# ghar1821/Chronoclust

Hardware: AMD Instinct MI355X
Metric: points clustered/sec (20-dim) (higher is better)
Workload: dtype f64; 1 GPU; C2: 1 timepoint, 1000000x20 synthetic blobs (seed 42+rank), 5000 microclusters; exact sequential semantics; online + offline phases per step; one independent st; points=1000000, dim=20, microclusters=5000, clusters=5000, streams=1

## Files before the change

### chronoclust_amd/_lib.py

```python
import ctypes as C
import os

import numpy as np

from . import build as _build

PCORE, OUTLIER = 0, 1
MAX_DIM = 1024

_ERRORS = {-1: "no HIP device / HIP runtime error", -2: "bad argument", -3: "non-finite input", -4: "out of memory",
           -5: "internal error", -6: "exchange between ranks failed"}


class ChronoclustHipError(RuntimeError):
    pass


class CcParams(C.Structure):
    _fields_ = [("eps_sq", C.c_double), ("delta_sq", C.c_double), ("k", C.c_double), ("beta", C.c_double),
                ("mu", C.c_double), ("omicron", C.c_double), ("ups_eps", C.c_double), ("ups_eps_sq", C.c_double),
                ("delta", C.c_double), ("pi", C.c_int32), ("pad", C.c_int32)]


class CcTuning(C.Structure):
# ... 165 lines not shown
        self._cofactors = None
        if transform is not None:
            if not isinstance(transform, ListTransform):
                raise ValueError("ListMode: transform must be a ListTransform")
            self._cofactors = transform.cofactors(self.shape[1])

    def __len__(self):
        return self.n

    def descriptor(self):
        return CcListMode(self._bytes.ctypes.data if self._bytes.size else None, self.n, self.src_cols,
                          LIST_DTYPES[self.dtype.newbyteorder("=")], LM_SWAPPED if self.swapped else 0, self.shape[1],
                          self.columns.ctypes.data_as(C.POINTER(C.c_int32)),
                          None if self.masks is None else self.masks.ctypes.data_as(C.POINTER(C.c_uint32)))

    def transform_descriptor(self):
        t = self.transform
        if t is None:
            return None
        return CcListTransform(t.m, 0, t.comp_cols.ctypes.data_as(C.POINTER(C.c_int32)) if t.m else None,
                               t.comp.ctypes.data_as(C.POINTER(C.c_double)) if t.m else None,
                               None if self._cofactors is None else self._cofactors.ctypes.data_as(C.POINTER(C.c_double)))

    def __array__(self, dtype=None, copy=None):
        rec = np.frombuffer(self._bytes, dtype=self.dtype, count=self.n * self.src_cols).reshape(self.n, self.src_cols)
        native = self.dtype.newbyteorder("=")
        out = rec[:, self.columns]
        if self.masks is not None:
            out = out.astype(native) & self.masks.astype(native)
        if self.transform is not None:
            out = self._host_transform(rec, out.astype(np.float64))
        else:
            out = out.astype(np.float32 if self.dtype.itemsize == 4 and self.dtype.kind == "f" else np.float64)
        return out if dtype is None else out.astype(dtype, copy=False)

    def _host_transform(self, rec, out):
        t = self.transform
        native = self.dtype.newbyteorder("=")
        cols = self.columns.tolist()
        xs = []
        for c in t.comp_cols.tolist():
            x = rec[:, c].astype(native)
            if self.masks is not None and c in cols:
                x = x & self.masks[cols.index(c)].astype(native)
            xs.append(x.astype(np.float64))
        for k, c in enumerate(cols):
            hit = np.flatnonzero(t.comp_cols == c)
            if hit.size:
                i = int(hit[0])
                v = xs[0] * t.comp[0, i]
                for j in range(1, t.m):
                    v = v + xs[j] * t.comp[j, i]
                out[:, k] = v
        if self._cofactors is not None:
            with np.errstate(all="ignore"):
                for k, cf in enumerate(self._cofactors.tolist()):
                    if cf > 0:
                        out[:, k] = np.arcsinh(out[:, k] / cf)
        return out


class CcRelaxedStats(C.Structure):
    _fields_ = [("super_steps", C.c_int64), ("minibatch_points", C.c_int64), ("deferred_points", C.c_int64),
                ("reserved", C.c_int64 * 5)]


_dp = C.POINTER(C.c_double)
_fp = C.POINTER(C.c_float)
_i64p = C.POINTER(C.c_int64)
_i32p = C.POINTER(C.c_int32)
_i8p = C.POINTER(C.c_int8)
_vp = C.POINTER(CcPointsView)
_lp = C.POINTER(CcListMode)
_xp = C.POINTER(CcListTransform)

SYMBOLS = {
    "cc_create": (C.c_int, [C.c_int, C.POINTER(C.c_void_p)]),
    "cc_destroy": (None, [C.c_void_p]),
    "cc_last_error": (C.c_char_p, [C.c_void_p]),
    "cc_set_tuning": (C.c_int, [C.c_void_p, C.POINTER(CcTuning)]),
    "cc_reset": (C.c_int, [C.c_void_p]),
    "cc_set_params": (C.c_int, [C.c_void_p, C.POINTER(CcParams)]),
    "cc_decay_downgrade": (C.c_int, [C.c_void_p, C.c_double]),
    "cc_points_upload": (C.c_int, [C.c_void_p, _dp, C.c_int64, C.c_int32]),
    "cc_points_prefetch": (C.c_int, [C.c_void_p, _dp, C.c_int64, C.c_int32, _dp, _dp]),
    "cc_online_run": (C.c_int, [C.c_void_p]),
    "cc_col_minmax": (C.c_int, [C.c_void_p, _dp, C.c_int64, C.c_int32, _dp, _dp]),
    "cc_points_upload_scaled": (C.c_int, [C.c_void_p, _dp, C.c_int64, C.c_int32, _dp, _dp]),
    "cc_points_download": (C.c_int, [C.c_void_p, _dp, _dp, _dp]),
    "cc_labels_download": (C.c_int, [C.c_void_p, _i64p, _i8p]),
    "cc_online": (C.c_int, [C.c_void_p, _dp, C.c_int64, C.c_int32, _i64p, _i8p]),
    "cc_assign": (C.c_int, [C.c_void_p, _dp, C.c_int64, C.c_int32, _i64p, _i8p, _dp]),
    "cc_points_upload_f32": (C.c_int, [C.c_void_p, _fp, C.c_int64, C.c_int32]),
    "cc_points_upload_scaled_f32": (C.c_int, [C.c_void_p, _fp, C.c_int64, C.c_int32, _dp, _dp]),
    "cc_points_prefetch_f32": (C.c_int, [C.c_void_p, _fp, C.c_int64, C.c_int32, _dp, _dp]),
    "cc_col_minmax_f32": (C.c_int, [C.c_void_p, _fp, C.c_int64, C.c_int32, _dp, _dp]),
    "cc_online_f32": (C.c_int, [C.c_void_p, _fp, C.c_int64, C.c_int32, _i64p, _i8p]),
    "cc_assign_f32": (C.c_int, [C.c_void_p, _fp, C.c_int64, C.c_int32, _i64p, _i8p, _dp]),
    "cc_points_download_xt": (C.c_int, [C.c_void_p, _dp]),
    "cc_f32_points": (C.c_int, [C.c_void_p, _i64p]),
    "cc_points_upload_view": (C.c_int, [C.c_void_p, _vp, _dp, _dp]),
    "cc_points_prefetch_view": (C.c_int, [C.c_void_p, _vp, _dp, _dp]),
    "cc_col_minmax_view": (C.c_int, [C.c_void_p, _vp, _dp, _dp]),
    "cc_online_view": (C.c_int, [C.c_void_p, _vp, _i64p, _i8p]),
    "cc_assign_view": (C.c_int, [C.c_void_p, _vp, _i64p, _i8p, _dp]),
    "cc_view_points": (C.c_int, [C.c_void_p, _i64p]),
    "cc_points_upload_list": (C.c_int, [C.c_void_p, _lp, _dp, _dp]),
    "cc_points_prefetch_list": (C.c_int, [C.c_void_p, _lp, _dp, _dp]),
    "cc_col_minmax_list": (C.c_int, [C.c_void_p, _lp, _dp, _dp]),
    "cc_online_list": (C.c_int, [C.c_void_p, _lp, _i64p, _i8p]),
    "cc_assign_list": (C.c_int, [C.c_void_p, _lp, _i64p, _i8p, _dp]),
    "cc_list_points": (C.c_int, [C.c_void_p, _i64p]),
    "cc_points_upload_list_xf": (C.c_int, [C.c_void_p, _lp, _xp, _dp, _dp]),
    "cc_points_prefetch_list_xf": (C.c_int, [C.c_void_p, _lp, _xp, _dp, _dp]),
    "cc_col_minmax_list_xf": (C.c_int, [C.c_void_p, _lp, _xp, _dp, _dp]),
    "cc_online_list_xf": (C.c_int, [C.c_void_p, _lp, _xp, _i64p, _i8p]),
    "cc_assign_list_xf": (C.c_int, [C.c_void_p, _lp, _xp, _i64p, _i8p, _dp]),
    "cc_count": (C.c_int, [C.c_void_p, C.c_int]),
    "cc_dim": (C.c_int, [C.c_void_p]),
    "cc_counters": (C.c_int, [C.c_void_p, _i64p, _i64p]),
    "cc_set_counters": (C.c_int, [C.c_void_p, C.c_int64, C.c_int64]),
    "cc_export": (C.c_int, [C.c_void_p, C.c_int, _i64p, _i64p, _dp, _dp, _dp, _dp, _dp]),
    "cc_inject_mc": (C.c_int, [C.c_void_p, C.c_int, C.c_int32, _dp, _dp, _dp, _dp, C.c_double, C.c_int64,
                               C.c_int64]),
    "cc_inject_bulk": (C.c_int, [C.c_void_p, C.c_int, C.c_int32, C.c_int32, _dp, _dp, _dp, _dp, _dp, _i64p, _i64p]),
    "cc_offline": (C.c_int, [C.c_void_p, _i32p, _i8p, _i32p, _i32p, _i32p]),
    "cc_num_core": (C.c_int, [C.c_void_p]),
    "cc_cluster_size": (C.c_int, [C.c_void_p, C.c_int32]),
    "cc_cluster_export": (C.c_int, [C.c_void_p, C.c_int32, _i64p, _dp, _dp, _dp, _dp, _dp]),
    "cc_clusters_total_members": (C.c_int, [C.c_void_p]),
    "cc_clusters_export": (C.c_int, [C.c_void_p, _i64p, _i32p, _dp, _dp, _dp, _dp, _dp]),
    "cc_assoc_argmin": (C.c_int, [C.c_void_p, _dp, _dp, C.c_int32, _dp, C.c_int32, C.c_int32, _i32p, _dp]),
    "cc_get_stats": (C.c_int, [C.c_void_p, C.POINTER(CcStats)]),
    "cc_sync": (C.c_int, [C.c_void_p]),
    "cc_policy_replay": (C.c_int, [C.POINTER(CcPolicyConfig), C.POINTER(CcPolicyCarry), C.c_int64, C.c_int32,
                                   C.POINTER(CcPolicyObs), C.c_int32, C.POINTER(CcPolicyDecision)]),
    "cc_point_clusters": (C.c_int, [C.c_void_p, _i32p]),
    "cc_format_points_csv": (C.c_int64, [_dp, C.c_int64, C.c_int32, C.c_int64, _i32p, C.c_char_p, _i32p, C.c_int32,
                                         C.c_void_p, C.c_int64]),
    "cc_comm_unique_id": (C.c_int, [C.c_char_p]),
    "cc_comm_init_rccl": (C.c_int, [C.c_void_p, C.c_char_p, C.c_int, C.c_int]),
    "cc_comm_init_local": (C.c_int, [C.POINTER(C.c_void_p), C.c_int]),
    "cc_comm_calibrate": (C.c_int, [C.c_void_p]),
    "cc_comm_destroy": (C.c_int, [C.c_void_p]),
    "cc_comm_info": (C.c_int, [C.c_void_p, _i32p, _i32p, _i32p]),
    "cc_comm_set_relaxed": (C.c_int, [C.c_void_p, C.c_int32]),
    "cc_get_relaxed_stats": (C.c_int, [C.c_void_p, C.POINTER(CcRelaxedStats)]),
    "cc_policy_seq_rate_guess": (C.c_double, [C.c_int32, C.c_int32, C.c_int32, C.c_int32]),
    "cc_seq_handover_replay": (C.c_int, [C.c_int32, C.c_int32, C.c_int32, C.POINTER(CcSeqEvent), C.c_int32, _i32p, _i64p]),
    "cc_batch_plan": (C.c_int, [C.POINTER(CcBatchInputs), C.POINTER(CcBatchGeometry)]),
    "cc_scan_width": (C.c_int, [C.c_int32, C.c_int32, C.c_int32, _i32p, _i32p, _i32p]),
    "cc_shard_rows": (C.c_int, [C.c_int32, C.c_int32, C.c_int32, C.c_int32, _i32p, _i32p]),
    "cc_set_shard_thresholds": (C.c_int, [C.c_void_p, C.c_int64, C.c_int32]),
}

COMM_ID_BYTES = 128

_lib = None


def load():
    global _lib
    if _lib is None:
        path = os.environ.get("CHRONOCLUST_HIP_LIB") or _build.LIB_PATH
        if not os.path.exists(path):
            raise ChronoclustHipError(
                "HIP library %s not built; run `python -m chronoclust_amd.build` (needs hipcc). "
                "chronoclust_amd has no CPU fallback." % path)
        if _build.is_stale(path) and os.environ.get("CHRONOCLUST_HIP_ALLOW_STALE") != "1":
            raise ChronoclustHipError(
                "HIP library %s was not built from the sources beside it (csrc/ or include/chronoclust_hip.h changed since, or "
                "its .sha256 stamp is missing); run `python -m chronoclust_amd.build`." % path)
        lib = C.CDLL(path)
        for name, (res, args) in SYMBOLS.items():
            fn = getattr(lib, name)
            fn.restype = res
            fn.argtypes = args
        _lib = lib
    return _lib


HOST_ONLY_SYMBOLS = ("cc_policy_replay", "cc_policy_seq_rate_guess", "cc_seq_handover_replay", "cc_batch_plan", "cc_shard_rows",
                     "cc_format_points_csv", "cc_scan_width")


def load_host_only(path):
    global _lib
    lib = C.CDLL(path)
    for name in HOST_ONLY_SYMBOLS:
        fn = getattr(lib, name)
        fn.restype, fn.argtypes = SYMBOLS[name]
    _lib = lib
    return lib


def _f64(a):
    return np.ascontiguousarray(np.asarray(a, dtype=np.float64))


def is_f32_points(a):
    return isinstance(a, np.ndarray) and a.dtype == np.float32 and a.ndim == 2 and a.flags["C_CONTIGUOUS"]


def as_points(a):
    return a if is_f32_points(a) else _f64(a)


def points_view(a):
    if not isinstance(a, np.ndarray) or a.ndim != 2 or a.shape[0] == 0 or a.shape[1] == 0:
        return None
    code = VIEW_DTYPES.get(a.dtype) if a.dtype.isnative else None
    if code is None:
        return None
    n, d = a.shape
    size = a.dtype.itemsize
    if a.strides[0] % size or a.strides[1] % size:
        return None
    rs, cs = a.strides[0] // size, a.strides[1] // size
    if d == 1:
        cs = 1
    if n == 1:
        rs = d if cs == 1 else 1
    if not ((cs == 1 and rs >= d) or (rs == 1 and cs >= n)):
        return None
    return CcPointsView(a.ctypes.data, n, d, code, rs, cs)


def points_source(a):
    if isinstance(a, np.ndarray) and a.ndim == 2 and a.flags["C_CONTIGUOUS"] and a.dtype in (np.float32, np.float64) \
            and a.dtype.isnative:
        return a, None
    view = points_view(a)
    if view is not None:
        return a, view
    return as_points(a), None


def xt_rows(d):
    return scan_width(d, False, False)[0] if 8 < d <= 64 else d


def _ptr(a, typ=_dp):
    return None if a is None else a.ctypes.data_as(typ)


def comm_unique_id():
    buf = C.create_string_buffer(COMM_ID_BYTES)
    rc = load().cc_comm_unique_id(buf)
    if rc != 0:
        raise ChronoclustHipError("cc_comm_unique_id failed (%s): is librccl available?" % _ERRORS.get(rc, rc))
    return buf.raw


def comm_init_local(handles):
    arr = (C.c_void_p * len(handles))(*[h._h for h in handles])
    rc = load().cc_comm_init_local(arr, len(handles))
    if rc != 0:
        raise ChronoclustHipError("cc_comm_init_local failed: %s" % _ERRORS.get(rc, rc))


def format_points_csv(values, first_id, label_idx, labels, threads=8, chunk=65536, out=None):
    from concurrent.futures import ThreadPoolExecutor
    lib = load()
    values = _f64(values)
    if values.ndim != 2:
        raise ValueError("values must be a [n, d] array, got shape %r" % (values.shape,))
    n, d = values.shape
    label_idx = np.ascontiguousarray(label_idx, dtype=np.int32)
    if label_idx.shape != (n,):
        raise ValueError("label_idx must hold one entry per row: shape %r for %d rows" % (label_idx.shape, n))
    if len(labels) < 1:
        raise ValueError("labels must not be empty")
    enc = [s.encode() for s in labels]
    offs = np.zeros(len(enc) + 1, np.int32)
    offs[1:] = np.cumsum([len(e) for e in enc])
    blob = b"".join(enc)
    per_row = 25 + max(len(e) for e in enc) + 33 * d + 2

    def work(a):
        b = min(n, a + chunk)
        buf = np.empty(per_row * (b - a), np.uint8)
        got = lib.cc_format_points_csv(values[a:b].ctypes.data_as(_dp), b - a, d, first_id + a,
                                       label_idx[a:b].ctypes.data_as(_i32p), blob, offs.ctypes.data_as(_i32p), len(enc),
                                       buf.ctypes.data, buf.size)
        if got < 0:
            raise ChronoclustHipError("cc_format_points_csv failed: %s" % _ERRORS.get(got, got))
        return memoryview(buf)[:got]

    if n == 0:
        return 0 if out is not None else b""
    starts = list(range(0, n, chunk))
    workers = max(1, threads)
    with ThreadPoolExecutor(max_workers=workers) as ex:
        if out is None:
            return b"".join(ex.map(work, starts))
        total, pending, nxt = 0, [], 0
        while nxt < len(starts) or pending:
            while nxt < len(starts) and len(pending) < 2 * workers:
                pending.append(ex.submit(work, starts[nxt]))
                nxt += 1
            part = pending.pop(0).result()
            out.write(part)
            total += len(part)
        return total


def policy_replay(config, carry, start, observations):
    cfg = CcPolicyConfig(**{k: int(v) for k, v in config.items()})
    car = CcPolicyCarry(int(carry[0]), int(carry[1]), int(carry[2]), 0)
    n = len(observations)
    obs = (CcPolicyObs * max(n, 1))()
    for i, o in enumerate(observations):
        for k, v in o.items():
            if k == "round_hist":
                for r, x in enumerate(v):
                    obs[i].round_hist[r] = int(x)
            else:
                setattr(obs[i], k, int(v))
    out = (CcPolicyDecision * (n + 1))()
    rc = load().cc_policy_replay(C.byref(cfg), C.byref(car), int(start[0]), int(start[1]), obs, n, out)
    if rc != 0:
        raise ValueError("cc_policy_replay: %s" % _ERRORS.get(rc, rc))
    keys = [k for k, _ in CcPolicyDecision._fields_ if k != "pad"]
    return [{k: getattr(d, k) for k in keys} for d in out], (car.adapt_win, car.clean_batches, car.since_shrink)


def seq_handover_replay(mode, possible, sticky, events):
    n = len(events)
    ev = (CcSeqEvent * max(n, 1))(*[CcSeqEvent(**e) for e in events])
    out, stint = (C.c_int32 * (n + 1))(), (C.c_int64 * (n + 1))()
    rc = load().cc_seq_handover_replay(int(mode), int(possible), int(sticky), ev, n, out, stint)
    if rc != 0:
        raise ValueError("cc_seq_handover_replay: %s" % _ERRORS.get(rc, rc))
    return list(out), list(stint)


def batch_plan(**inputs):
    out = CcBatchGeometry()
    rc = load().cc_batch_plan(C.byref(CcBatchInputs(**inputs)), C.byref(out))
    if rc != 0:
        raise ValueError("cc_batch_plan(%r): %s" % (inputs, _ERRORS.get(rc, rc)))
    return {k: getattr(out, k) for k, _ in CcBatchGeometry._fields_ if k != "pad"}


SCAN_CHAINS = ("none", "common", "general")


def scan_width(d, filter_on, k_pow2):
    padded, scan_u, chain = C.c_int32(), C.c_int32(), C.c_int32()
    rc = load().cc_scan_width(int(d), int(bool(filter_on)), int(bool(k_pow2)), C.byref(padded), C.byref(scan_u), C.byref(chain))
    if rc != 0:
        raise ValueError("cc_scan_width(%r, %r, %r): %s" % (d, filter_on, k_pow2, _ERRORS.get(rc, rc)))
    return padded.value, bool(scan_u.value), SCAN_CHAINS[chain.value]


def shard_rows(n, world, rank, unit=1):
    lo, hi = C.c_int32(), C.c_int32()
    rc = load().cc_shard_rows(int(n), int(world), int(rank), int(unit), C.byref(lo), C.byref(hi))
    if rc != 0:
        raise ValueError("cc_shard_rows(%r, %r, %r, %r): %s" % (n, world, rank, unit, _ERRORS.get(rc, rc)))
    return lo.value, hi.value


_DESCRIBED = ("view", "list", "list_xf")
_INGEST = {
    "upload": {"f64": "cc_points_upload", "f32": "cc_points_upload_f32",
               "view": "cc_points_upload_view", "list": "cc_points_upload_list", "list_xf": "cc_points_upload_list_xf"},
    "upload_scaled": {"f64": "cc_points_upload_scaled", "f32": "cc_points_upload_scaled_f32",
                      "view": "cc_points_upload_view", "list": "cc_points_upload_list", "list_xf": "cc_points_upload_list_xf"},
    "prefetch": {"f64": "cc_points_prefetch", "f32": "cc_points_prefetch_f32",
                 "view": "cc_points_prefetch_view", "list": "cc_points_prefetch_list", "list_xf": "cc_points_prefetch_list_xf"},
    "col_minmax": {"f64": "cc_col_minmax", "f32": "cc_col_minmax_f32",
                   "view": "cc_col_minmax_view", "list": "cc_col_minmax_list", "list_xf": "cc_col_minmax_list_xf"},
    "assign": {"f64": "cc_assign", "f32": "cc_assign_f32", "view": "cc_assign_view", "list": "cc_assign_list",
               "list_xf": "cc_assign_list_xf"},
}
_SCALED_REFUSAL = "points must be [n, d], scale and min_ [d]"


class Handle(object):

    def __init__(self, device=0):
        self._lib = load()
        h = C.c_void_p()
        rc = self._lib.cc_create(int(device), C.byref(h))
        if rc != 0:
            raise ChronoclustHipError("cc_create(device=%d) failed: %s. chronoclust_amd needs an MI355X-class HIP "
                                      "device; there is no CPU fallback." % (device, _ERRORS.get(rc, rc)))
        self._h = h
        self.device = device
        self._prefetched = None

    def close(self):
        if getattr(self, "_h", None):
            self._lib.cc_destroy(self._h)
            self._h = None

    def __del__(self):
        try:
            self.close()
        except Exception:
            pass

    def _check(self, rc):
        if rc < 0:
            msg = self._lib.cc_last_error(self._h)
            exc = ValueError if rc in (-2, -3) else ChronoclustHipError
            raise exc("%s: %s" % (_ERRORS.get(rc, rc), msg.decode() if msg else ""))
        return rc

    def set_tuning(self, window=0, rounds=0, segments=0, windows_per_sync=0, time_kernels=0, dirty_segments=0,
                   lookahead=0, early_window=0, sequential=0):
        t = CcTuning(window, rounds, segments, windows_per_sync, time_kernels, dirty_segments, int(early_window),
                     int(lookahead), int(sequential))
        self._check(self._lib.cc_set_tuning(self._h, C.byref(t)))

    def reset(self):
        self._check(self._lib.cc_reset(self._h))

    def set_params(self, eps_sq, delta_sq, k, beta, mu, omicron, ups_eps, ups_eps_sq, delta, pi):
        p = CcParams(eps_sq, delta_sq, k, beta, mu, omicron, ups_eps, ups_eps_sq, delta, int(pi), 0)
        self._check(self._lib.cc_set_params(self._h, C.byref(p)))

    def decay_downgrade(self, factor):
        self._check(self._lib.cc_decay_downgrade(self._h, float(factor)))

    def _source(self, x, refusal="points must be a 2-d array"):
        if isinstance(x, ListMode):
            desc, xf = x.descriptor(), x.transform_descriptor()
            if xf is not None:
                return ("list_xf", x, (C.byref(desc), C.byref(xf))) + x.shape
            return ("list", x, (C.byref(desc),)) + x.shape
        x, view = points_source(x)
        if x.ndim != 2:
            raise ValueError(refusal)
        if view is not None:
            return ("view", x, (C.byref(view),)) + x.shape
        f32 = x.dtype == np.float32
        return ("f32" if f32 else "f64", x, (_ptr(x, _fp if f32 else _dp),) + x.shape) + x.shape

    def _ingest(self, op, kind, *args):
        self._check(getattr(self._lib, _INGEST[op][kind])(self._h, *args))

    def _upload(self, x, scale, min_):
        kind, x, args, n, d = self._source(x, "points must be a 2-d array" if scale is None else _SCALED_REFUSAL)
        op = "upload"
        if scale is not None:
            op, scale, min_ = "upload_scaled", _f64(scale), _f64(min_)
            if scale.shape != (d,) or min_.shape != (d,):
                raise ValueError(_SCALED_REFUSAL)
        if scale is not None or kind in _DESCRIBED:
            args += (_ptr(scale), _ptr(min_))
        try:
            self._ingest(op, kind, *args)
        finally:
            self._prefetched = None
        self._n = n

    def points_upload(self, x):
        self._upload(x, None, None)

    def points_upload_scaled(self, x, scale, min_):
        self._upload(x, scale, min_)

    def points_prefetch(self, x, scale=None, min_=None):
        if isinstance(x, (np.ndarray, ListMode)) and x.ndim == 2 and x.shape[0] == 0:
            return
        refusal = ("points_prefetch needs an [n, d] array that is taken as it lies - C-contiguous float64 or float32, "
                   "or a layout and element type points_view accepts (it is not copied)")
        kind, src, args, n, d = self._source(x, refusal)
        if src is not x:
            raise ValueError(refusal)
        scale = None if scale is None else _f64(scale)
        min_ = None if min_ is None else _f64(min_)
        self._prefetched = (x, scale, min_)
        self._ingest("prefetch", kind, *(args + (_ptr(scale), _ptr(min_))))

    def col_minmax(self, x):
        kind, x, args, n, d = self._source(x)
        mn = np.empty(d, dtype=np.float64)
        mx = np.empty(d, dtype=np.float64)
        self._ingest("col_minmax", kind, *(args + (_ptr(mn), _ptr(mx))))
        return mn, mx

    def points_download(self, d, scale=None, min_=None):
        out = np.empty((self._n, d), dtype=np.float64)
        if scale is None:
            self._check(self._lib.cc_points_download(self._h, _ptr(out), None, None))
        else:
            scale, min_ = _f64(scale), _f64(min_)
            self._check(self._lib.cc_points_download(self._h, _ptr(out), _ptr(scale), _ptr(min_)))
        return out

    def points_download_xt(self, d):
        out = np.empty((xt_rows(d), self._n), dtype=np.float64)
        self._check(self._lib.cc_points_download_xt(self._h, _ptr(out)))
        return out

    def online_run(self):
        self._check(self._lib.cc_online_run(self._h))

    def labels_download(self, want_path=True):
        uid = np.empty(self._n, dtype=np.int64)
        path = np.empty(self._n, dtype=np.int8) if want_path else None
        self._check(self._lib.cc_labels_download(self._h, _ptr(uid, _i64p), _ptr(path, _i8p)))
        return uid, path

    def online(self, x):
        self.points_upload(x)
        self.online_run()
        return self.labels_download()

    def assign(self, x, want_path=True, want_dist=False):
        kind, x, args, n, d = self._source(x)
        uid = np.empty(n, dtype=np.int64)
        path = np.empty(n, dtype=np.int8) if want_path else None
# ... 144 lines not shown
```

### chronoclust_amd/csrc/cc_api.hip

```cpp
#include <hip/hip_runtime.h>

#include <algorithm>
#include <chrono>
#include <cmath>
#include <cstdio>
#include <cstdlib>
#include <cstring>
#include <limits>
#include <optional>
#include <string>
#include <thread>
#include <type_traits>
#include <vector>

#include "../../include/chronoclust_hip.h"
#include "cc_comm.h"
#include "cc_common.h"
#include "cc_csv.h"
#include "cc_offline.h"
#include "cc_online.h"
#include "cc_assign.h"
#include "cc_policy.h"
#include "cc_batch.h"

// ... 212 lines not shown
                ++h->stats.scan_g_launches;
                unsigned long long* const found = h->lean_now ? nullptr : h->found.p;
                if (h->group_guess_now) {
                    hipLaunchKernelGGL(k_pstat_zero, dim3(1), dim3(2), 0, st, (const Ctl*)h->ctl.p, h->pstat_p(), round, mode);
                    return window_scan(shard_rank, shard_world, h->prune_F, found, false);
                }
                window_scan(0, 1, h->prune_F, found, false);
                if (h->lean_now) { ++h->stats.scan_lean_launches; return; }
                hipLaunchKernelGGL(k_missed, dim3(1), dim3(1024), 0, st, h->ctl.p, h->found.p, h->missed.p, CC_MISSED_CAP, round, mode);
                return missed_scan(h->missed.p);
            }
        }
        if (pl.scan_u) return L.scan_u(win, shard_rank, shard_world, nullptr);
    }
    const bool filter = DIRTY || h->hc.filter != 0;
#define CC_LAUNCH_SCAN(F, P) hipLaunchKernelGGL((k_scan<DP, F, P, DIRTY, NW>), grid, block, 0, st, h->ctl.p, h->X.p, h->Xt.p, rows, clean, \
                                          part, round, mode, h->part_stride, shard_rank, shard_world)
    if (filter) {
        if (h->hc.pow2) CC_LAUNCH_SCAN(true, true);
        else CC_LAUNCH_SCAN(true, false);
    } else if constexpr (!DIRTY) {
        if (h->hc.pow2) CC_LAUNCH_SCAN(false, true);
        else CC_LAUNCH_SCAN(false, false);
    }
#undef CC_LAUNCH_SCAN
}

template <bool DIRTY>
void launch_scan(cc_handle* h, hipStream_t st, int win, Rows rows, const Cand* clean, Cand* part, int S, int round,
                 int mode, int shard_rank = 0, int shard_world = 1, int phase = 0)
{
#define CC_SCAN_DP(DP) return launch_scan_dp<DP, DIRTY>(h, st, win, rows, clean, part, S, round, mode, shard_rank, shard_world, phase)
    switch (h->scan_plan.dp) {
    case 4: CC_SCAN_DP(4);
    case 8: CC_SCAN_DP(8);
    case 14: CC_SCAN_DP(14);
    case 16: CC_SCAN_DP(16);
    case 20: CC_SCAN_DP(20);
    case 32: CC_SCAN_DP(32);
    case 40: CC_SCAN_DP(40);
    case 64: CC_SCAN_DP(64);
    }
    throw HipErr{hipErrorInvalidValue, "launch_scan before scan_plan() (OnlineRun::prepare)"};
#undef CC_SCAN_DP
}

Rows padded_rows(cc_handle* h, hipStream_t st, Rows rows, int q, int round, int mode)
{
    const int dp = h->scan_plan.dp;
    ensure_pad_rows(h, dp);
    double* const cen = h->pad_cen.p + (size_t)q * h->pad_stride;
    double* const scl = h->pad_scl.p + (size_t)q * h->pad_stride;
    const dim3 grid((unsigned)((h->tab.cap * (size_t)(dp / 2) + 255) / 256));
#define CC_PAD_DP(DP) hipLaunchKernelGGL((k_pad_rows<DP>), grid, dim3(256), 0, st, (const Ctl*)h->ctl.p, rows.cen, rows.scl, cen, scl, \
                                         h->d, round, mode); break
    switch (dp) {
    case 14: CC_PAD_DP(14);
    case 16: CC_PAD_DP(16);
    case 20: CC_PAD_DP(20);
    case 32: CC_PAD_DP(32);
    case 40: CC_PAD_DP(40);
    case 64: CC_PAD_DP(64);
    default: throw HipErr{hipErrorInvalidValue, "padded_rows: no scan over padded operands at this width"};
    }
#undef CC_PAD_DP
    ++h->stats.pad_rows_launches;
    rows.cen = cen;
    rows.scl = scl;
    return rows;
}

}

#include "cc_online_run.h"
#include "cc_api_points.inc"
#include "cc_api_views.inc"
#include "cc_api_list.inc"
#include "cc_api_ingest.inc"
#include "cc_api_offline.inc"
#include "cc_api_comm.inc"
#include "cc_api_assign.inc"


extern "C" {

int cc_create(int device, cc_handle** out)
{
    if (!out) return CC_ERR_BAD_ARG;
    *out = nullptr;
    int ndev = 0;
    if (hipGetDeviceCount(&ndev) != hipSuccess || ndev <= 0 || device < 0 || device >= ndev) return CC_ERR_NO_DEVICE;
    cc_handle* h = new (std::nothrow) cc_handle();
    if (!h) return CC_ERR_OOM;
    h->device = device;
    int rc = guarded(h, [&]() {
        int prio_lo = 0, prio_hi = 0;
        int cus = 0;
        if (hipDeviceGetAttribute(&cus, hipDeviceAttributeMultiprocessorCount, device) == hipSuccess && cus > 0) h->n_cus = cus;
        HIPCHK(hipDeviceGetStreamPriorityRange(&prio_lo, &prio_hi));
        HIPCHK(hipStreamCreateWithPriority(&h->stream, hipStreamNonBlocking, prio_hi));
        HIPCHK(hipStreamCreateWithPriority(&h->stream2, hipStreamNonBlocking, prio_lo));
        h->ctl.ensure(1);
        if (hipHostMalloc((void**)&h->hc_pin, 2 * sizeof(Ctl), hipHostMallocDefault) != hipSuccess) h->hc_pin = nullptr;
        h->badflag.ensure(4);
        memset(&h->hc, 0, sizeof(Ctl));
        h->tun.window = CC_MAX_WINDOW;
        h->tun.rounds = 3;
        h->tun.segments = 64;
        h->tun.windows_per_sync = 16;
        h->tun.time_kernels = 0;
        read_knobs(*h);
        push_ctl(h);
        sync_stream(h, h->stream);
        return CC_OK;
    });
    if (rc != CC_OK) {
        delete h;
        return rc;
    }
    *out = h;
    return CC_OK;
}

void cc_destroy(cc_handle* h)
{
    if (!h) return;
    (void)hipSetDevice(h->device);
    if (h->pf.worker.joinable()) h->pf.worker.join();
    if (h->pf.stream) (void)hipStreamDestroy(h->pf.stream);
    if (h->hc_pin) (void)hipHostFree(h->hc_pin);
    for (int q = 0; q < 2; ++q)
        if (h->pf.pin[q]) (void)hipHostFree(h->pf.pin[q]);
    auto drain = [&](hipStream_t st) {
        if (!st) return;
        try {
            if (h->comm.rccl() && !h->comm.broken) h->comm.wait_stream(st);
            else (void)hipStreamSynchronize(st);
        } catch (const cc::CommErr&) {
        }
    };
    drain(h->stream);
    drain(h->stream2);
    h->comm.destroy();
    if (h->stream) {
        (void)hipStreamSynchronize(h->stream);
        (void)hipStreamDestroy(h->stream);
    }
    if (h->stream2) {
        (void)hipStreamSynchronize(h->stream2);
        (void)hipStreamDestroy(h->stream2);
    }
    for (hipEvent_t e : h->ev_pool) (void)hipEventDestroy(e);
    for (hipEvent_t e : h->sync_pool) (void)hipEventDestroy(e);
    delete h;
}

const char* cc_last_error(const cc_handle* h) { return h ? h->err.c_str() : "null handle"; }

int cc_set_tuning(cc_handle* h, const cc_tuning* t)
{
    if (!h || !t) return CC_ERR_BAD_ARG;
    if (t->window > 0) h->tun.window = std::min(t->window, CC_MAX_WINDOW);
    if (t->rounds > 0) h->tun.rounds = std::min(t->rounds, CC_MAX_ROUNDS);
    if (t->segments > 0) h->tun.segments = std::min(t->segments, 1024);
    if (t->windows_per_sync > 0) h->tun.windows_per_sync = t->windows_per_sync;
    h->tun.time_kernels = t->time_kernels;
    if (t->dirty_segments > 0) h->tun.dirty_segments = std::min(t->dirty_segments, 1024);
    h->tun.lookahead = t->lookahead;
    h->tun.sequential = t->sequential;
    if (t->early_window > 0) h->tun.early_window = t->early_window;
    return CC_OK;
}

int cc_reset(cc_handle* h)
{
    if (!h) return CC_ERR_BAD_ARG;
    return guarded(h, [&]() {
        Ctl& c = h->hc;
        c.m_rows = 0;
        c.n_pkeys = c.n_okeys = 0;
        c.pcore_last_id = c.outlier_last_id = 0;
        c.cursor = 0;
        h->tainted = false;
        h->adapt_win = 0;
        h->seq_sticky = false;
        h->clean_batches = 0;
        h->since_shrink = 1000;
        h->clusters.clear();
        h->n_core = 0;
        refresh_ctl_params(h);
        push_ctl(h);
        sync_stream(h, h->stream);
        return (int)CC_OK;
    });
}

int cc_set_params(cc_handle* h, const cc_params* p)
{
    if (!h || !p) return CC_ERR_BAD_ARG;
    if (h->have_par && h->hc.m_rows > 0 && p->k != h->par.k) h->tainted = true;
    h->par = *p;
    h->have_par = true;
    refresh_ctl_params(h);
    return CC_OK;
}

int cc_dim(cc_handle* h) { return h ? h->d : CC_ERR_BAD_ARG; }

int cc_counters(cc_handle* h, int64_t* pcore_last_id, int64_t* outlier_last_id)
{
    if (!h) return CC_ERR_BAD_ARG;
    if (pcore_last_id) *pcore_last_id = h->hc.pcore_last_id;
    if (outlier_last_id) *outlier_last_id = h->hc.outlier_last_id;
    return CC_OK;
}

int cc_set_counters(cc_handle* h, int64_t pcore_last_id, int64_t outlier_last_id)
{
    if (!h || pcore_last_id < 0 || outlier_last_id < 0) return CC_ERR_BAD_ARG;
    return guarded(h, [&]() {
        h->hc.pcore_last_id = pcore_last_id;
        h->hc.outlier_last_id = outlier_last_id;
        push_ctl(h);
        sync_stream(h, h->stream);
        return (int)CC_OK;
    });
}

int cc_online_run(cc_handle* h)
{
    if (!h) return CC_ERR_BAD_ARG;
    if (!h->have_par) return fail(h, CC_ERR_BAD_ARG, "cc_set_params has not been called");
    return guarded(h, [&]() {
        memset(&h->stats, 0, sizeof(h->stats));
        if (h->relaxed_minibatch > 0 && h->comm.active()) return online_relaxed(h);
        return online_range(h, 0, h->n_points, false, false);
    });
}

int cc_labels_download(cc_handle* h, int64_t* out_uid, int8_t* out_path)
{
    if (!h) return CC_ERR_BAD_ARG;
    return guarded(h, [&]() {
        const size_t n = (size_t)h->n_points;
        if (n == 0) return (int)CC_OK;
        static_assert(sizeof(long long) == sizeof(int64_t), "int64");
        if (out_uid) HIPCHK(hipMemcpyAsync(out_uid, h->lab_uid.p, n * 8, hipMemcpyDeviceToHost, h->stream));
        if (out_path) HIPCHK(hipMemcpyAsync(out_path, h->lab_path.p, n, hipMemcpyDeviceToHost, h->stream));
        sync_stream(h, h->stream);
        return (int)CC_OK;
    });
}

int cc_online(cc_handle* h, const double* x, int64_t n, int32_t d, int64_t* out_uid, int8_t* out_path)
{
    int rc = cc_points_upload(h, x, n, d);
    if (rc != CC_OK) return rc;
    rc = cc_online_run(h);
    if (rc != CC_OK) return rc;
    return cc_labels_download(h, out_uid, out_path);
}

int cc_online_f32(cc_handle* h, const float* x, int64_t n, int32_t d, int64_t* out_uid, int8_t* out_path)
{
    int rc = cc_points_upload_f32(h, x, n, d);
    if (rc != CC_OK) return rc;
    rc = cc_online_run(h);
    if (rc != CC_OK) return rc;
    return cc_labels_download(h, out_uid, out_path);
}

int cc_count(cc_handle* h, int kind)
{
    if (!h) return CC_ERR_BAD_ARG;
    int n = 0;
    int rc = guarded(h, [&]() {
        RowList rl = list_order(h);
        n = (int)(kind == CC_PCORE ? rl.pcore.size() : rl.outlier.size());
        return (int)CC_OK;
    });
    return rc == CC_OK ? n : rc;
}

int cc_export(cc_handle* h, int kind, int64_t* id, int64_t* uid, double* w, double* cf1, double* cf2, double* cen,
              double* pref)
{
    if (!h) return CC_ERR_BAD_ARG;
    return guarded(h, [&]() {
        RowList rl = list_order(h);
        const std::vector<int>& rows = kind == CC_PCORE ? rl.pcore : rl.outlier;
        const size_t m = (size_t)h->hc.m_rows, d = (size_t)h->d, n = rows.size();
        if (n == 0) return (int)CC_OK;
        auto fetch_vec = [&](const double* dev, double* out) {
            if (!out) return;
            std::vector<double> tmp(m * d);
            HIPCHK(hipMemcpyAsync(tmp.data(), dev, m * d * 8, hipMemcpyDeviceToHost, h->stream));
            sync_stream(h, h->stream);
            for (size_t i = 0; i < n; ++i) memcpy(out + i * d, tmp.data() + (size_t)rows[i] * d, d * 8);
        };
        fetch_vec(h->tab.cf1.p, cf1);
        fetch_vec(h->tab.cf2.p, cf2);
        fetch_vec(h->tab.cen.p, cen);
        fetch_vec(h->tab.pref.p, pref);
        if (w) {
            std::vector<double> tmp(m);
            HIPCHK(hipMemcpyAsync(tmp.data(), h->tab.w.p, m * 8, hipMemcpyDeviceToHost, h->stream));
            sync_stream(h, h->stream);
            for (size_t i = 0; i < n; ++i) w[i] = tmp[rows[i]];
        }
        auto fetch_i64 = [&](const long long* dev, int64_t* out) {
            if (!out) return;
            std::vector<long long> tmp(m);
            HIPCHK(hipMemcpyAsync(tmp.data(), dev, m * 8, hipMemcpyDeviceToHost, h->stream));
            sync_stream(h, h->stream);
            for (size_t i = 0; i < n; ++i) out[i] = tmp[rows[i]];
        };
        fetch_i64(h->tab.id.p, id);
        fetch_i64(h->tab.uid.p, uid);
        return (int)CC_OK;
    });
}

int cc_inject_mc(cc_handle* h, int kind, int32_t d, const double* cf1, const double* cf2, const double* cen,
                 const double* pref, double w, int64_t id, int64_t uid)
{
    if (!h || !cf1 || !cf2 || !cen || !pref) return CC_ERR_BAD_ARG;
    return guarded(h, [&]() {
        int rc = set_dim(h, d);
        if (rc != CC_OK) return rc;
        ensure_table(h, (size_t)h->hc.m_rows + 1);
        const size_t r = (size_t)h->hc.m_rows, dd = (size_t)d;
        for (int i = 0; i < d; ++i)
            if (pref[i] != 1.0 && !(h->have_par && pref[i] == h->par.k)) h->tainted = true;
        HIPCHK(hipMemcpyAsync(h->tab.cf1.p + r * dd, cf1, dd * 8, hipMemcpyHostToDevice, h->stream));
        HIPCHK(hipMemcpyAsync(h->tab.cf2.p + r * dd, cf2, dd * 8, hipMemcpyHostToDevice, h->stream));
        HIPCHK(hipMemcpyAsync(h->tab.cen.p + r * dd, cen, dd * 8, hipMemcpyHostToDevice, h->stream));
        HIPCHK(hipMemcpyAsync(h->tab.pref.p + r * dd, pref, dd * 8, hipMemcpyHostToDevice, h->stream));
        const int knd = kind == CC_PCORE ? CC_KIND_PCORE : CC_KIND_OUTLIER;
        const int key = kind == CC_PCORE ? h->hc.n_pkeys++ : h->hc.n_okeys++;
        const long long lid = id, luid = uid;
        HIPCHK(hipMemcpyAsync(h->tab.w.p + r, &w, 8, hipMemcpyHostToDevice, h->stream));
        HIPCHK(hipMemcpyAsync(h->tab.kind.p + r, &knd, 4, hipMemcpyHostToDevice, h->stream));
        HIPCHK(hipMemcpyAsync(h->tab.key.p + r, &key, 4, hipMemcpyHostToDevice, h->stream));
        HIPCHK(hipMemcpyAsync(h->tab.id.p + r, &lid, 8, hipMemcpyHostToDevice, h->stream));
        HIPCHK(hipMemcpyAsync(h->tab.uid.p + r, &luid, 8, hipMemcpyHostToDevice, h->stream));
// ... 93 lines not shown
```

### chronoclust_amd/csrc/cc_api_offline.inc

```

namespace {

struct RowList {
    std::vector<int> pcore, outlier;
};

RowList list_order(cc_handle* h, std::vector<int>* kind_out = nullptr, std::vector<int>* key_out = nullptr)
{
    const int m = h->hc.m_rows;
    std::vector<int> kind(m), key(m);
    if (m) {
        HIPCHK(hipMemcpyAsync(kind.data(), h->tab.kind.p, (size_t)m * 4, hipMemcpyDeviceToHost, h->stream));
        HIPCHK(hipMemcpyAsync(key.data(), h->tab.key.p, (size_t)m * 4, hipMemcpyDeviceToHost, h->stream));
        sync_stream(h, h->stream);
    }
    RowList rl;
    for (int r = 0; r < m; ++r) {
        if (kind[r] == CC_KIND_PCORE) rl.pcore.push_back(r);
        else if (kind[r] == CC_KIND_OUTLIER) rl.outlier.push_back(r);
    }
    auto by_key = [&](int a, int b) { return key[a] < key[b]; };
    std::sort(rl.pcore.begin(), rl.pcore.end(), by_key);
    std::sort(rl.outlier.begin(), rl.outlier.end(), by_key);
    if (kind_out) *kind_out = kind;
    if (key_out) *key_out = key;
    return rl;
}

}

extern "C" {

int cc_decay_downgrade(cc_handle* h, double factor)
{
    if (!h) return CC_ERR_BAD_ARG;
    if (!h->have_par) return fail(h, CC_ERR_BAD_ARG, "cc_set_params has not been called");
    return guarded(h, [&]() {
        const int m = h->hc.m_rows, d = h->d;
        if (m == 0) return (int)CC_OK;
        refresh_ctl_params(h);
        const Table tab = h->tab.view();
        hipLaunchKernelGGL(k_decay, dim3((m * d + 255) / 256), dim3(256), 0, h->stream, tab, m, d, factor);
        h->flags.ensure((size_t)m);
        hipLaunchKernelGGL(k_downgrade_flags, dim3((m + 255) / 256), dim3(256), 0, h->stream, tab, m, d,
                           h->hc.beta_mu, h->hc.pi, h->hc.omicron, h->flags.p);
        std::vector<int> flags(m);
        std::vector<long long> id(m), uid(m);
        HIPCHK(hipMemcpyAsync(flags.data(), h->flags.p, (size_t)m * 4, hipMemcpyDeviceToHost, h->stream));
        HIPCHK(hipMemcpyAsync(id.data(), tab.id, (size_t)m * 8, hipMemcpyDeviceToHost, h->stream));
        HIPCHK(hipMemcpyAsync(uid.data(), tab.uid, (size_t)m * 8, hipMemcpyDeviceToHost, h->stream));
        RowList rl = list_order(h);

        std::vector<int> pl = rl.pcore, ol = rl.outlier;
        std::vector<char> downgraded(m, 0);
        for (size_t i = 0; i < pl.size(); ++i) {
            const int r = pl[i];
            if (flags[r] & 1) {
                downgraded[r] = 1;
                pl.erase(pl.begin() + (long)i);
                ol.push_back(r);
            }
        }
        for (size_t i = 0; i < ol.size(); ++i) {
            if (flags[ol[i]] & 2) ol.erase(ol.begin() + (long)i);
        }
        const int np = (int)pl.size(), no = (int)ol.size(), n = np + no;
        std::vector<int> perm(n), nkind(n), nkey(n);
        std::vector<long long> nid(n);
        for (int i = 0; i < np; ++i) { perm[i] = pl[i]; nkind[i] = CC_KIND_PCORE; nkey[i] = i; nid[i] = id[pl[i]]; }
        for (int i = 0; i < no; ++i) {
            const int r = ol[i];
            perm[np + i] = r; nkind[np + i] = CC_KIND_OUTLIER; nkey[np + i] = i;
            nid[np + i] = downgraded[r] ? uid[r] : id[r];
        }
        if (h->tab2.cap < h->tab.cap || h->tab2.d != d) {
            h->tab2.alloc(h->tab.cap, d);
            HIPCHK(hipMemsetAsync(h->tab2.touch.p, 0, 2 * h->tab2.cap * 8, h->stream));
            HIPCHK(hipMemsetAsync(h->tab2.last.p, 0, 2 * h->tab2.cap * 8, h->stream));
            HIPCHK(hipMemsetAsync(h->tab2.carry_of.p, 0, h->tab2.cap * 8, h->stream));
            HIPCHK(hipMemsetAsync(h->tab2.cnt.p, 0, h->tab2.cap * 8, h->stream));
        }
        DevBuf<int> dperm, dkind, dkey;
        DevBuf<long long> dnid;
        dperm.ensure(n); dkind.ensure(n); dkey.ensure(n); dnid.ensure(n);
        if (n) {
            HIPCHK(hipMemcpyAsync(dperm.p, perm.data(), (size_t)n * 4, hipMemcpyHostToDevice, h->stream));
            HIPCHK(hipMemcpyAsync(dkind.p, nkind.data(), (size_t)n * 4, hipMemcpyHostToDevice, h->stream));
            HIPCHK(hipMemcpyAsync(dkey.p, nkey.data(), (size_t)n * 4, hipMemcpyHostToDevice, h->stream));
            HIPCHK(hipMemcpyAsync(dnid.p, nid.data(), (size_t)n * 8, hipMemcpyHostToDevice, h->stream));
            hipLaunchKernelGGL(k_gather_rows, dim3((n * d + 255) / 256), dim3(256), 0, h->stream, tab, h->tab2.view(),
                               dperm.p, dkind.p, dkey.p, dnid.p, n, d);
        }
        sync_stream(h, h->stream);
        std::swap(h->tab, h->tab2);
        h->hc.m_rows = n;
        h->hc.n_pkeys = np;
        h->hc.n_okeys = no;
        push_ctl(h);
        sync_stream(h, h->stream);
        return (int)CC_OK;
    });
}

int cc_offline(cc_handle* h, int32_t* n_clusters, int8_t* out_core, int32_t* out_pdim, int32_t* out_nn,
               int32_t* out_nw)
{
    if (!h) return CC_ERR_BAD_ARG;
    if (!h->have_par) return fail(h, CC_ERR_BAD_ARG, "cc_set_params has not been called");
    return guarded(h, [&]() {
        refresh_ctl_params(h);
        h->clusters.clear();
        h->pcore_ids_host.clear();
        h->pcore_uid_host.clear();
        h->n_core = 0;
        if (n_clusters) *n_clusters = 0;
        auto now_us = []() { return std::chrono::duration<double, std::micro>(std::chrono::steady_clock::now().time_since_epoch()).count(); };
        double tph[8] = {now_us(), 0, 0, 0, 0, 0, 0, 0};
        const int m_all = h->hc.m_rows;
        h->pin.reset();
        h->pin.reserve((size_t)m_all * 72 + ((size_t)1 << 16));
        std::vector<int> prow_host;
        const long long* uid_all = nullptr;
        if (m_all > 0) {
            int* kind = h->pin.take<int>((size_t)m_all);
            int* key = h->pin.take<int>((size_t)m_all);
            long long* uid = h->pin.take<long long>((size_t)m_all);
            HIPCHK(hipMemcpyAsync(kind, h->tab.kind.p, (size_t)m_all * 4, hipMemcpyDeviceToHost, h->stream));
            HIPCHK(hipMemcpyAsync(key, h->tab.key.p, (size_t)m_all * 4, hipMemcpyDeviceToHost, h->stream));
            HIPCHK(hipMemcpyAsync(uid, h->tab.uid.p, (size_t)m_all * 8, hipMemcpyDeviceToHost, h->stream));
            sync_stream(h, h->stream);
            uid_all = uid;
            std::vector<unsigned long long> order;
            order.reserve((size_t)m_all);
            for (int r = 0; r < m_all; ++r)
                if (kind[r] == CC_KIND_PCORE) order.push_back(((unsigned long long)((unsigned)key[r] ^ 0x80000000u) << 32) | (unsigned)r);
            std::sort(order.begin(), order.end());
            prow_host.resize(order.size());
            for (size_t i = 0; i < order.size(); ++i) prow_host[i] = (int)(order[i] & 0xFFFFFFFFull);
        }
        tph[1] = now_us();
        const int mp = (int)prow_host.size(), d = h->d;
        if (mp == 0) return (int)CC_OK;
        const size_t md = (size_t)mp * d;
        const int words = (mp + 63) / 64;
        const int world = h->comm.world, rank = h->comm.rank;
        const bool shard = h->comm.active() && mp >= h->offline_shard_min_rows;
        const int share = shard ? cc_shard_share(mp, world, 64) : words * 64;
        const size_t rows_pad = shard ? (size_t)share * world : (size_t)mp;
        int p_lo = 0, p_hi = mp;
        if (shard) cc_shard_range(mp, world, rank, 64, &p_lo, &p_hi);
        h->pv_cf1.ensure(md); h->pv_cf2.ensure(md); h->pv_cen.ensure(md); h->pv_pref.ensure(md); h->pv_w.ensure(mp);
        h->pv_id.ensure(mp); h->prow.ensure(mp); h->wvec.ensure(rows_pad * d); h->nn.ensure(rows_pad); h->pdim.ensure(mp);
        h->core.ensure(mp); h->adj.ensure(rows_pad * words); h->adjw.ensure(rows_pad * words);
        int* const prow_pin = h->pin.take<int>((size_t)mp);
        memcpy(prow_pin, prow_host.data(), (size_t)mp * 4);
        HIPCHK(hipMemcpyAsync(h->prow.p, prow_pin, (size_t)mp * 4, hipMemcpyHostToDevice, h->stream));
        PcoreView pv{h->pv_cf1.p, h->pv_cf2.p, h->pv_cen.p, h->pv_pref.p, h->pv_w.p, h->pv_id.p};
        const Ctl& c = h->hc;
        const cc_params& p = h->par;
        hipLaunchKernelGGL(k_gather_pcores, dim3((unsigned)((md + 255) / 256)), dim3(256), 0, h->stream, h->tab.view(),
                           pv, h->prow.p, mp, d);
        hipLaunchKernelGGL(k_core_flags, dim3((mp + 255) / 256), dim3(256), 0, h->stream, pv, mp, d, p.eps_sq, p.mu,
                           p.pi, p.k, c.inv_k, c.pow2, h->core.p);
        const int my_rows = p_hi - p_lo;
        if (my_rows > 0) {
            {
                int pch = CC_EPS_PCH;
                while (pch > CC_EPS_TP && (long long)((words + 3) / 4) * ((my_rows + pch - 1) / pch) < 8ll * h->n_cus) pch /= 2;
                const dim3 grid((words + 3) / 4, (my_rows + pch - 1) / pch), block(256);
#define CC_EPS(DP) hipLaunchKernelGGL((k_eps_neighbours<DP>), grid, block, 0, h->stream, pv.cen, mp, d, p.ups_eps, h->adj.p, words, p_lo, p_hi, pch)
                if (d <= 4) CC_EPS(4);
                else if (d <= 8) CC_EPS(8);
                else if (d <= 16) CC_EPS(16);
                else if (d <= 20) CC_EPS(20);
                else if (d <= 24) CC_EPS(24);
                else if (d <= 40) CC_EPS(40);
                else if (d <= 64) CC_EPS(64);
                else if (d <= 128) CC_EPS(128);
                else hipLaunchKernelGGL(k_eps_neighbours_blk, grid, block, 0, h->stream, pv.cen, mp, d, p.ups_eps, h->adj.p, words,
                                        p_lo, p_hi, pch);
#undef CC_EPS
            }
            hipLaunchKernelGGL(k_subspace_pref, dim3((unsigned)(((size_t)my_rows * d + 255) / 256)), dim3(256), 0, h->stream,
                               pv.cen, h->adj.p, words, mp, d, p.delta, p.k, h->wvec.p, h->nn.p, p_lo, p_hi);
        }
        if (shard) {
            h->comm.all_gather(h->wvec.p + (size_t)rank * share * d, h->wvec.p, (size_t)share * d * 8, h->stream);
            h->comm.all_gather(h->nn.p + (size_t)rank * share, h->nn.p, (size_t)share * 4, h->stream);
        }
        hipLaunchKernelGGL(k_pdim, dim3((mp + 255) / 256), dim3(256), 0, h->stream, h->wvec.p, mp, d, h->pdim.p);
        if (my_rows > 0)
            hipLaunchKernelGGL(k_weighted_reach, dim3(my_rows), dim3(64), 0, h->stream, pv.cen, h->wvec.p, h->adj.p,
                               h->adjw.p, words, mp, d, p.ups_eps_sq, p_lo, p_hi);
        if (shard)
            h->comm.all_gather(h->adjw.p + (size_t)rank * share * words, h->adjw.p, (size_t)share * words * 8, h->stream);
        h->nw_cnt.ensure(mp);
        hipLaunchKernelGGL(k_adj_counts, dim3(mp), dim3(64), 0, h->stream, h->adjw.p, words, mp, h->nw_cnt.p);
        h->pcore_uid_host.resize(mp);
        for (int i = 0; i < mp; ++i) h->pcore_uid_host[(size_t)i] = uid_all[(size_t)prow_host[(size_t)i]];
        int8_t* const core = h->pin.take<int8_t>((size_t)mp);
        int* const pdim = h->pin.take<int>((size_t)mp);
        int* const nn = h->pin.take<int>((size_t)mp);
        int* const nw_cnt = h->pin.take<int>((size_t)mp);
        long long* const ids_pin = h->pin.take<long long>((size_t)mp);
        long long* const nw_off = h->pin.take<long long>((size_t)mp + 1);
        HIPCHK(hipMemcpyAsync(core, h->core.p, mp, hipMemcpyDeviceToHost, h->stream));
        HIPCHK(hipMemcpyAsync(pdim, h->pdim.p, (size_t)mp * 4, hipMemcpyDeviceToHost, h->stream));
        HIPCHK(hipMemcpyAsync(nn, h->nn.p, (size_t)mp * 4, hipMemcpyDeviceToHost, h->stream));
        HIPCHK(hipMemcpyAsync(nw_cnt, h->nw_cnt.p, (size_t)mp * 4, hipMemcpyDeviceToHost, h->stream));
        HIPCHK(hipMemcpyAsync(ids_pin, h->pv_id.p, (size_t)mp * 8, hipMemcpyDeviceToHost, h->stream));
        sync_stream(h, h->stream);
        HIPCHK(hipGetLastError());
        h->pcore_ids_host.assign(ids_pin, ids_pin + mp);
        tph[2] = now_us();
        nw_off[0] = 0;
        for (int i = 0; i < mp; ++i) nw_off[(size_t)i + 1] = nw_off[i] + nw_cnt[i];
        const long long n_edges = nw_off[mp];
        std::vector<int> nbr_pageable;
        const int* nbr = nullptr;
        if (n_edges > 0) {
            h->nw_off.ensure((size_t)mp + 1);
            h->nw_nbr.ensure((size_t)n_edges);
            HIPCHK(hipMemcpyAsync(h->nw_off.p, nw_off, ((size_t)mp + 1) * 8, hipMemcpyHostToDevice, h->stream));
            hipLaunchKernelGGL(k_adj_fill, dim3(mp), dim3(64), 0, h->stream, h->adjw.p, words, mp, h->nw_off.p, h->nw_nbr.p);
            int* dst;
            if (h->pin.used + (size_t)n_edges * 4 + 128 <= h->pin.cap) dst = h->pin.take<int>((size_t)n_edges);
            else {
                nbr_pageable.resize((size_t)n_edges);
                dst = nbr_pageable.data();
            }
            HIPCHK(hipMemcpyAsync(dst, h->nw_nbr.p, (size_t)n_edges * 4, hipMemcpyDeviceToHost, h->stream));
            sync_stream(h, h->stream);
            HIPCHK(hipGetLastError());
            nbr = dst;
        }

        tph[3] = now_us();
        auto for_each_nw = [&](int q, auto&& fn) {
            for (long long e = nw_off[q]; e < nw_off[(size_t)q + 1]; ++e) fn(nbr[(size_t)e]);
        };
        std::vector<int8_t> cls(mp, 0);
        std::vector<int> queue;
        h->clusters.mem.reserve((size_t)mp);
        h->clusters.off.reserve((size_t)mp + 1);
        const int lam = p.pi;
        for (int seed = 0; seed < mp; ++seed) {
            if (cls[seed] != 0) continue;
            if (!core[seed]) { cls[seed] = 2; continue; }
            const size_t cl_begin = h->clusters.mem.size();
            queue.clear();
            for_each_nw(seed, [&](int x) { queue.push_back(x); });
            size_t head = 0;
            while (head < queue.size()) {
                const int q = queue[head++];
                if (!core[q]) continue;
                for_each_nw(q, [&](int x) {
                    if (pdim[x] > lam) return;
                    if (cls[x] == 0) queue.push_back(x);
                    if (cls[x] == 0 || cls[x] == 2) {
                        cls[x] = 1;
                        h->clusters.mem.push_back(x);
                    }
                });
            }
            if (h->clusters.mem.size() > cl_begin) h->clusters.off.push_back((int)h->clusters.mem.size());
        }
        for (int i = 0; i < mp; ++i) h->n_core += core[i];

        tph[4] = now_us();
        const int nc = (int)h->clusters.size();
        if (nc) {
            const std::vector<int>&mem = h->clusters.mem, &off = h->clusters.off;
            const size_t cd = (size_t)nc * d;
            h->mem_dev.ensure(mem.size()); h->off_dev.ensure(off.size());
            h->c_cf1.ensure(cd); h->c_cf2.ensure(cd); h->c_cen.ensure(cd); h->c_pref.ensure(cd); h->c_w.ensure(nc);
            HIPCHK(hipMemcpyAsync(h->mem_dev.p, mem.data(), mem.size() * 4, hipMemcpyHostToDevice, h->stream));
            HIPCHK(hipMemcpyAsync(h->off_dev.p, off.data(), off.size() * 4, hipMemcpyHostToDevice, h->stream));
            hipLaunchKernelGGL(k_cluster_merge, dim3((unsigned)((cd + 255) / 256)), dim3(256), 0, h->stream, pv,
                               h->mem_dev.p, h->off_dev.p, nc, d, p.delta_sq, p.k, h->c_cf1.p, h->c_cf2.p, h->c_cen.p,
                               h->c_pref.p, h->c_w.p);
            sync_stream(h, h->stream);
        }
        tph[5] = now_us();
        if (h->trace)
            fprintf(stderr, "[cc] offline phase, host wall time: list order %.0f us, pair kernels + read-back %.0f, neighbour lists %.0f, "
                    "ordered expansion %.0f, cluster sums %.0f (%d pcores, %d clusters)\n", tph[1] - tph[0], tph[2] - tph[1], tph[3] - tph[2],
                    tph[4] - tph[3], tph[5] - tph[4], mp, nc);
        if (out_core) memcpy(out_core, core, mp);
        if (out_pdim) memcpy(out_pdim, pdim, (size_t)mp * 4);
        if (out_nn) memcpy(out_nn, nn, (size_t)mp * 4);
        if (out_nw) memcpy(out_nw, nw_cnt, (size_t)mp * 4);
        if (n_clusters) *n_clusters = nc;
        return (int)CC_OK;
    });
}

int cc_num_core(cc_handle* h) { return h ? h->n_core : CC_ERR_BAD_ARG; }

int cc_cluster_size(cc_handle* h, int32_t c)
{
    if (!h || c < 0 || c >= (int)h->clusters.size()) return CC_ERR_BAD_ARG;
    return h->clusters.off[(size_t)c + 1] - h->clusters.off[(size_t)c];
}

int cc_cluster_export(cc_handle* h, int32_t c, int64_t* members, double* w, double* cf1, double* cf2, double* cen,
                      double* pref)
{
    if (!h || c < 0 || c >= (int)h->clusters.size()) return CC_ERR_BAD_ARG;
    return guarded(h, [&]() {
        const size_t d = (size_t)h->d;
        const int a = h->clusters.off[(size_t)c], e = h->clusters.off[(size_t)c + 1];
        if (members)
            for (int i = a; i < e; ++i) members[i - a] = h->pcore_ids_host[(size_t)h->clusters.mem[(size_t)i]];
        if (w) HIPCHK(hipMemcpyAsync(w, h->c_w.p + c, 8, hipMemcpyDeviceToHost, h->stream));
        if (cf1) HIPCHK(hipMemcpyAsync(cf1, h->c_cf1.p + (size_t)c * d, d * 8, hipMemcpyDeviceToHost, h->stream));
        if (cf2) HIPCHK(hipMemcpyAsync(cf2, h->c_cf2.p + (size_t)c * d, d * 8, hipMemcpyDeviceToHost, h->stream));
        if (cen) HIPCHK(hipMemcpyAsync(cen, h->c_cen.p + (size_t)c * d, d * 8, hipMemcpyDeviceToHost, h->stream));
        if (pref) HIPCHK(hipMemcpyAsync(pref, h->c_pref.p + (size_t)c * d, d * 8, hipMemcpyDeviceToHost, h->stream));
        sync_stream(h, h->stream);
        return (int)CC_OK;
    });
}

int cc_clusters_total_members(cc_handle* h)
{
    if (!h) return CC_ERR_BAD_ARG;
    size_t tot = 0;
    tot = h->clusters.mem.size();
    return (int)tot;
}

int cc_clusters_export(cc_handle* h, int64_t* members, int32_t* offsets, double* w, double* cf1, double* cf2,
                       double* cen, double* pref)
{
    if (!h) return CC_ERR_BAD_ARG;
    return guarded(h, [&]() {
        const size_t nc = h->clusters.size(), d = (size_t)h->d;
        const size_t tot = h->clusters.mem.size();
        if (offsets)
            for (size_t c = 0; c <= nc; ++c) offsets[c] = (int32_t)h->clusters.off[c];
        if (members)
            for (size_t i = 0; i < tot; ++i) members[i] = h->pcore_ids_host[(size_t)h->clusters.mem[i]];
        if (nc == 0) return (int)CC_OK;
        if (w) HIPCHK(hipMemcpyAsync(w, h->c_w.p, nc * 8, hipMemcpyDeviceToHost, h->stream));
        if (cf1) HIPCHK(hipMemcpyAsync(cf1, h->c_cf1.p, nc * d * 8, hipMemcpyDeviceToHost, h->stream));
        if (cf2) HIPCHK(hipMemcpyAsync(cf2, h->c_cf2.p, nc * d * 8, hipMemcpyDeviceToHost, h->stream));
        if (cen) HIPCHK(hipMemcpyAsync(cen, h->c_cen.p, nc * d * 8, hipMemcpyDeviceToHost, h->stream));
        if (pref) HIPCHK(hipMemcpyAsync(pref, h->c_pref.p, nc * d * 8, hipMemcpyDeviceToHost, h->stream));
        sync_stream(h, h->stream);
        return (int)CC_OK;
    });
}

int cc_assoc_argmin(cc_handle* h, const double* cur_cen, const double* cur_pref, int32_t mc, const double* prev_cen,
                    int32_t mp, int32_t d, int32_t* out_idx, double* out_dist)
{
    if (!h || !cur_cen || !cur_pref || !out_idx || mc < 0 || mp < 0 || d <= 0) return CC_ERR_BAD_ARG;
    if (mp > 0 && !prev_cen) return CC_ERR_BAD_ARG;
    return guarded(h, [&]() {
        if (mc == 0) return (int)CC_OK;
        const size_t cd = (size_t)mc * d, pd = (size_t)mp * d;
        const int world = h->comm.world, rank = h->comm.rank;
        const bool shard = h->comm.active() && mc >= h->offline_shard_min_rows;
        const int share = shard ? cc_shard_share(mc, world, 1) : mc;
        int c_lo = 0, c_hi = mc;
        if (shard) cc_shard_range(mc, world, rank, 1, &c_lo, &c_hi);
        h->a_cur_cen.ensure(cd); h->a_cur_pref.ensure(cd); h->a_prev_cen.ensure(pd);
        h->a_idx.ensure(shard ? (size_t)share * world : (size_t)mc);
        h->a_dist.ensure(shard ? (size_t)share * world : (size_t)mc);
        const double k = h->have_par ? h->par.k : 1.0;
        bool unit = is_pow2(k);
        for (size_t i = 0; unit && i < cd; ++i) unit = cur_pref[i] == 1.0 || cur_pref[i] == k;
        std::vector<double> op(cd);
        const double inv_k = unit ? 1.0 / k : 0.0;
        for (size_t i = 0; i < cd; ++i) op[i] = unit ? (cur_pref[i] == 1.0 ? 1.0 : inv_k) : cur_pref[i];
        HIPCHK(hipMemcpyAsync(h->a_cur_cen.p, cur_cen, cd * 8, hipMemcpyHostToDevice, h->stream));
        HIPCHK(hipMemcpyAsync(h->a_cur_pref.p, op.data(), cd * 8, hipMemcpyHostToDevice, h->stream));
        if (pd) HIPCHK(hipMemcpyAsync(h->a_prev_cen.p, prev_cen, pd * 8, hipMemcpyHostToDevice, h->stream));
        if (c_hi > c_lo && mp > 0) {
            const int ctiles = (c_hi - c_lo + 255) / 256;
            const int S = std::max(1, std::min((mp + CC_ASSOC_TQ - 1) / CC_ASSOC_TQ, (1024 + ctiles - 1) / ctiles));
            h->a_pdist.ensure((size_t)S * mc);
            h->a_pidx.ensure((size_t)S * mc);
            const dim3 grid(ctiles, S), block(256);
            auto assoc = [&](auto DP) {
                with_bools([&](auto UNIT) {
                    hipLaunchKernelGGL((k_assoc_tiled<decltype(DP)::value, decltype(UNIT)::value>), grid, block, 0, h->stream,
                                       h->a_cur_cen.p, h->a_cur_pref.p, h->a_prev_cen.p, mc, mp, d, c_lo, c_hi, h->a_pdist.p, h->a_pidx.p);
                }, unit);
            };
            if (d <= 4) assoc(std::integral_constant<int, 4>{});
            else if (d <= 8) assoc(std::integral_constant<int, 8>{});
            else if (d <= 16) assoc(std::integral_constant<int, 16>{});
            else if (d <= 24) assoc(std::integral_constant<int, 24>{});
            else if (d <= 40) assoc(std::integral_constant<int, 40>{});
            else if (d <= 64) assoc(std::integral_constant<int, 64>{});
            else if (d <= 128) assoc(std::integral_constant<int, 128>{});
            else
                with_bools([&](auto UNIT) {
                    hipLaunchKernelGGL((k_assoc_tiled_blk<decltype(UNIT)::value>), grid, block, 0, h->stream, h->a_cur_cen.p,
                                       h->a_cur_pref.p, h->a_prev_cen.p, mc, mp, d, c_lo, c_hi, h->a_pdist.p, h->a_pidx.p);
                }, unit);
            hipLaunchKernelGGL(k_assoc_merge, dim3((c_hi - c_lo + 255) / 256), dim3(256), 0, h->stream, h->a_pdist.p,
                               h->a_pidx.p, S, mc, c_lo, c_hi, h->a_idx.p, h->a_dist.p);
        } else if (c_hi > c_lo) {
            HIPCHK(hipMemsetAsync(h->a_idx.p + c_lo, 0xFF, (size_t)(c_hi - c_lo) * 4, h->stream));
            const std::vector<double> inf((size_t)(c_hi - c_lo), std::numeric_limits<double>::infinity());
            HIPCHK(hipMemcpyAsync(h->a_dist.p + c_lo, inf.data(), inf.size() * 8, hipMemcpyHostToDevice, h->stream));
            HIPCHK(hipStreamSynchronize(h->stream));
        }
        if (shard) {
            h->comm.all_gather(h->a_idx.p + (size_t)rank * share, h->a_idx.p, (size_t)share * 4, h->stream);
            h->comm.all_gather(h->a_dist.p + (size_t)rank * share, h->a_dist.p, (size_t)share * 8, h->stream);
        }
        HIPCHK(hipMemcpyAsync(out_idx, h->a_idx.p, (size_t)mc * 4, hipMemcpyDeviceToHost, h->stream));
        if (out_dist) HIPCHK(hipMemcpyAsync(out_dist, h->a_dist.p, (size_t)mc * 8, hipMemcpyDeviceToHost, h->stream));
        sync_stream(h, h->stream);
        HIPCHK(hipGetLastError());
        return (int)CC_OK;
    });
}


int cc_point_clusters(cc_handle* h, int32_t* out_idx)
{
    if (!h || !out_idx) return CC_ERR_BAD_ARG;
    return guarded(h, [&]() {
        const long long n = h->n_points;
        if (n == 0) return (int)CC_OK;
        const long long n_uid = h->hc.outlier_last_id;
        std::vector<int32_t> map((size_t)std::max<long long>(n_uid, 1), -1);
        for (size_t c = 0; c < h->clusters.size(); ++c)
            for (int i = h->clusters.off[c]; i < h->clusters.off[c + 1]; ++i) {
                const long long u = h->pcore_uid_host[(size_t)h->clusters.mem[(size_t)i]];
                if (u >= 0 && u < n_uid) map[(size_t)u] = (int32_t)c;
            }
        h->pc_map.ensure(map.size());
        h->pc_out.ensure((size_t)n);
        HIPCHK(hipMemcpyAsync(h->pc_map.p, map.data(), map.size() * 4, hipMemcpyHostToDevice, h->stream));
        hipLaunchKernelGGL(k_point_clusters, dim3((unsigned)((n + 255) / 256)), dim3(256), 0, h->stream, h->lab_uid.p, n,
                           h->pc_map.p, n_uid, h->pc_out.p);
        HIPCHK(hipMemcpyAsync(out_idx, h->pc_out.p, (size_t)n * 4, hipMemcpyDeviceToHost, h->stream));
        sync_stream(h, h->stream);
        HIPCHK(hipGetLastError());
        return (int)CC_OK;
    });
}

}
```

### chronoclust_amd/csrc/cc_handle.h

```cpp
#pragma once
#include "cc_knobs.h"
#include "cc_ingest_src.h"

namespace {

struct HipErr {
    hipError_t e;
    const char* what;
};

#define HIPCHK(call)                                  \
    do {                                              \
        hipError_t _e = (call);                       \
        if (_e != hipSuccess) throw HipErr{_e, #call}; \
    } while (0)

template <typename T>
struct DevBuf {
    T* p = nullptr;
    size_t n = 0;
    void ensure(size_t count)
    {
        if (count <= n && p) return;
        release();
// ... 24 lines not shown
    {
        std::swap(p, o.p);
        std::swap(n, o.n);
    }
};

struct TableStore {
    DevBuf<double> cf1, cf2, cen, pref, scl, w;
    DevBuf<int> kind, key;
    DevBuf<long long> id, uid;
    DevBuf<unsigned long long> touch, last, carry_of, cnt;
    DevBuf<int> memb, clen, heavy;
    size_t cap = 0;
    int d = 0;
    enum Grow { KEPT, CLEARED, CLEARED_KEPT, SCRATCH };
    template <typename F>
    static void for_each_column(int dims, F&& f)
    {
        const size_t dim = (size_t)dims;
        f(&TableStore::cf1, dim, KEPT); f(&TableStore::cf2, dim, KEPT); f(&TableStore::cen, dim, KEPT);
        f(&TableStore::pref, dim, KEPT); f(&TableStore::scl, dim, KEPT);
        f(&TableStore::w, (size_t)1, KEPT); f(&TableStore::kind, (size_t)1, KEPT); f(&TableStore::key, (size_t)1, KEPT);
        f(&TableStore::id, (size_t)1, KEPT); f(&TableStore::uid, (size_t)1, KEPT);
        f(&TableStore::touch, (size_t)2, CLEARED); f(&TableStore::last, (size_t)2, CLEARED);
        f(&TableStore::carry_of, (size_t)1, CLEARED_KEPT);
        f(&TableStore::cnt, (size_t)1, CLEARED); f(&TableStore::memb, (size_t)CC_CHAIN_MEMB, SCRATCH);
        f(&TableStore::clen, (size_t)1, CLEARED);
        f(&TableStore::heavy, (size_t)1, CLEARED_KEPT);
    }
    void alloc(size_t rows, int dim)
    {
        for_each_column(dim, [&](auto col, size_t per_row, Grow) { (this->*col).ensure(rows * per_row); });
        cap = rows;
        d = dim;
    }
    Table view() const { return Table{cf1.p, cf2.p, cen.p, pref.p, scl.p, w.p, kind.p, key.p, id.p, uid.p, touch.p, last.p, carry_of.p, cnt.p, memb.p, clen.p, heavy.p, cap}; }
};

struct HostClusters {
    std::vector<int> mem, off{0};
    size_t size() const { return off.size() - 1; }
    void clear() { mem.clear(); off.assign(1, 0); }
};

}

struct PinArena {
    char* p = nullptr;
    size_t cap = 0, used = 0;
    void reset() { used = 0; }
    void reserve(size_t bytes)
    {
        if (bytes <= cap) return;
        if (p) (void)hipHostFree(p);
        p = nullptr;
        cap = 0;
        const size_t want = std::max<size_t>(bytes, (size_t)1 << 20);
        if (hipHostMalloc((void**)&p, want, hipHostMallocDefault) != hipSuccess) {
            p = nullptr;
            throw HipErr{hipErrorOutOfMemory, "hipHostMalloc"};
        }
        cap = want;
    }
    template <typename T>
    T* take(size_t n)
    {
        used = (used + 63) & ~(size_t)63;
        T* r = reinterpret_cast<T*>(p + used);
        used += std::max<size_t>(n, 1) * sizeof(T);
        if (used > cap) throw HipErr{hipErrorOutOfMemory, "page-locked scratch exhausted"};
        return r;
    }
    ~PinArena() { if (p) (void)hipHostFree(p); }
    PinArena() = default;
    PinArena(const PinArena&) = delete;
    PinArena& operator=(const PinArena&) = delete;
};

struct ScanPlan {
    int dp = 0;
    bool scan_u = false;
    bool pad_rows = false;
    enum Chain { NONE, COMMON, GENERAL } chain = NONE;
    enum Form { P3, P2, P1 } form = P1;
    long long split_rows = std::numeric_limits<long long>::max(), listed_rows = 0;
    bool seed16 = false;
    int prune_applicable = 0, allow_guess = 0, allow_probe = 0, force_prune_rows = 0;
    int waves = 4, dirty_waves = 4;
    int plain_wgs_per_cu = 1, prune_wgs_per_cu = 1;
    bool split(long long m_rows) const { return m_rows >= split_rows; }
    bool listed(long long m_rows) const { return m_rows >= listed_rows; }
};


struct BatchScanState {
    bool prune_now = false;
    bool group_guess_now = false;
    bool lean_now = false;
    bool guess_now = false;
    bool probe_now = false;
    ScanPlan scan_plan;
    void set_prune(int prune)
    {
        prune_now = prune != 0;
        guess_now = prune >= 2;
        lean_now = prune == 3;
    }
};

struct PrunedScanBuffers {
    DevBuf<Cand> probe_part;
    DevBuf<unsigned long long> found;
    DevBuf<int> missed;
    DevBuf<SeedCand> spart;
    DevBuf<double> thr;
    DevBuf<float> thr32;
    DevBuf<unsigned long long> cmax;
    DevBuf<cc_h8> a16;
    DevBuf<Prefix16Hdr> hdr16;
    size_t a16_stride = 0;
    DevBuf<unsigned> masks;
    size_t mask_stride = 0;
    DevBuf<double> pad_cen, pad_scl;
    size_t pad_stride = 0;
    size_t spart_stride = 0, thr_stride = 0;
};

struct WindowBuffers {
    int win_alloc = 0, seg_alloc = 0, d_alloc = 0;
    DevBuf<double> v_cf1, v_cf2, v_cen, v_pref, v_scl, v_w, v_dsq, v_tau;
    DevBuf<unsigned long long> v_tile_dsq;
    DevBuf<int> v_kind, v_key, v_next, v_upg, v_acc, v_tgt, v_skip, v_skip_car, v_unsafe;
    DevBuf<Cand> part, clean, dpart, dpart2, dseed;
    size_t part_stride = 0;
    DevBuf<double> c_cf1v, c_cf2v, c_cenv, c_prefv, c_sclv, c_wv, c_c0, c_w0, c_dsq;
    DevBuf<int> c_kind, c_key, c_slot, c_kind0;
    DevBuf<unsigned long long> c_tile_dsq;
    DevBuf<int> T0, T1, rk;
    DevBuf<int> link_near;
    DevBuf<int> sp_list;
    DevBuf<int> long_list;
    DevBuf<unsigned long long> lstat, lprev;
    bool prep_launched = false;
    DevBuf<CommitRec> rec;
    DevBuf<double> sh_cen[2], sh_scl[2], sh_cf1[2], sh_cf2[2], sh_w[2];
    DevBuf<int> sh_kind[2], sh_key[2];
    DevBuf<int8_t> dpath;
};

struct OfflineResults {
    DevBuf<double> pv_cf1, pv_cf2, pv_cen, pv_pref, pv_w, wvec;
    DevBuf<long long> pv_id;
    DevBuf<int> prow, nn, pdim, mem_dev, off_dev, nw_cnt, nw_nbr;
    DevBuf<long long> nw_off;
    DevBuf<int8_t> core;
    DevBuf<unsigned long long> adj, adjw;
    DevBuf<double> c_cf1, c_cf2, c_cen, c_pref, c_w;
    HostClusters clusters;
    PinArena pin;
    std::vector<long long> pcore_ids_host, pcore_uid_host;
    DevBuf<int32_t> pc_map, pc_out;
    int n_core = 0;
};

struct AssocScratch {
    DevBuf<double> a_cur_cen, a_cur_pref, a_prev_cen, a_dist, a_pdist;
    DevBuf<int> a_idx, a_pidx;
    DevBuf<int> flags;
};

struct RelaxedState {
    int relaxed_minibatch = 0;
    bool shard_suspended = false;
    DevBuf<double> rs_cf1, rs_cf2, rs_w, r_delta, r_gather;
    DevBuf<int> rs_kind, rs_key, r_didx, r_didx_all, r_cnt_all;
    DevBuf<long long> rs_id;
    DevBuf<double> rg_X, rg_Xt;
    DevBuf<long long> rg_uid;
    DevBuf<int8_t> rg_path;
    cc_relaxed_stats rstats{};
};

struct AssignBuffers {
    struct Set {
        DevBuf<double> X, Xt, dist;
        DevBuf<float> raw;
        DevBuf<long long> uid;
        DevBuf<int8_t> path;
        DevBuf<Cand> part;
        DevBuf<int> bad;
    } asg[2];
};

struct cc_handle : Knobs, BatchScanState, PrunedScanBuffers, WindowBuffers, OfflineResults, AssocScratch, RelaxedState, AssignBuffers {
    int device = 0;
    hipStream_t stream = nullptr;
    hipStream_t stream2 = nullptr;
    std::string err;
    cc_params par{};
    bool have_par = false;
    cc_tuning tun{};
    cc_stats stats{};

    int d = 0;
    TableStore tab, tab2;
    Ctl hc{};
    Ctl* hc_pin = nullptr;
    DevBuf<Ctl> ctl;
    unsigned long long* pstat_p() const { return (unsigned long long*)((char*)ctl.p + offsetof(Ctl, pstat)); }
    bool tainted = false;
    int adapt_win = 0;
    int clean_batches = 0;
    int since_shrink = 1000;
    DevBuf<int> seq_lists;
    DevBuf<double> seq_img;
    bool seq_sticky = false;
    int n_cus = 256;

    DevBuf<double> X, Xt;
    long long n_points = 0;
    double x_absmax = 0.0;
    DevBuf<long long> lab_uid;
    DevBuf<int8_t> lab_path;
    DevBuf<int> badflag;
    DevBuf<double> scr, scr2;
    DevBuf<float> ingest_raw[2];
    long long f32_points = 0;
    long long view_points = 0;
    long long list_points = 0;
    DevBuf<int> list_desc;

    struct Prefetch {
        std::thread worker;
        bool active = false;
        IngestSrc src;
        bool scaled = false;
        long long piece = 0;
        DevBuf<int> desc;
        DevBuf<float> raw[2];
        std::vector<double> scale, mn;
        DevBuf<double> X, Xt, sm;
        DevBuf<int> bad;
        hipStream_t stream = nullptr;
        void* pin[2] = {nullptr, nullptr};
        size_t pin_bytes = 0;
        int bad_host[4] = {0, 0, 0, 0};
        int rc = 0;
        const char* what = "";
    } pf;

    std::vector<hipEvent_t> ev_pool, sync_pool;

    cc::Comm comm;
    long long shard_min_row_dims = 400000;
    long long shard_min_row_dims_pruned = 0;
    double calib_ag_us = 0.0, calib_scan_ns = 0.0;
    int offline_shard_min_rows = 8192;
    DevBuf<Cand> gsend, gpart;
    DevBuf<Cand> gsend2, gpart2;
    size_t gsend_stride = 0, gpart_stride = 0;
    DevBuf<int> g_i32;
};

namespace {

template <typename F>
void with_bools(F&& f)
{
    f();
}
template <typename F, typename... Rest>
void with_bools(F&& f, bool b, Rest... rest)
{
    if (b) with_bools([&](auto... c) { f(std::true_type{}, c...); }, rest...);
    else with_bools([&](auto... c) { f(std::false_type{}, c...); }, rest...);
}

struct CapacityErr {
    std::string what;
};

int fail(cc_handle* h, int code, const std::string& msg)
{
    if (h) h->err = msg;
    return code;
}

void group_lost(cc_handle* h)
{
    if (h && h->comm.active()) h->comm.fail_group();
}

template <typename F>
int guarded(cc_handle* h, F&& f)
{
    try {
        if (h) HIPCHK(hipSetDevice(h->device));
        const int rc = f();
        if (rc < 0) group_lost(h);
        return rc;
    } catch (const HipErr& e) {
        char buf[512];
        snprintf(buf, sizeof buf, "HIP error %d (%s) in %s", (int)e.e, hipGetErrorString(e.e), e.what);
        group_lost(h);
        return fail(h, e.e == hipErrorOutOfMemory ? CC_ERR_OOM : CC_ERR_NO_DEVICE, buf);
    } catch (const cc::CommErr& e) {
        group_lost(h);
        return fail(h, CC_ERR_COMM, "exchange between ranks failed: " + e.what);
    } catch (const std::bad_alloc&) {
        group_lost(h);
// ... 219 lines not shown
```

### chronoclust_amd/csrc/cc_host.h

```cpp
#pragma once
#include <stdint.h>

#if defined(__HIPCC__) || defined(__HIP__)
#define CC_HOSTDEV __host__ __device__
#else
#define CC_HOSTDEV
#endif

CC_HOSTDEV inline int cc_shard_share(int n, int world, int unit)
{
    const long long units = ((long long)n + unit - 1) / unit;
    const long long share = ((units + world - 1) / world) * unit;
    return (int)(share < 0x7fffffffLL ? share : 0x7fffffffLL);
}
CC_HOSTDEV inline void cc_shard_range(int n, int world, int rank, int unit, int* lo, int* hi)
{
    const int share = cc_shard_share(n, world, unit);
    const long long a = (long long)rank * share;
    *lo = (int)(a < n ? a : n);
    const long long b = a + share;
    *hi = (int)(b < n ? b : n);
}

#define CC_SEQ_DOUBLES 6600
CC_HOSTDEV inline int cc_seq_cap_rows(int d) { return CC_SEQ_DOUBLES / (4 * d + 5); }
```

### chronoclust_amd/csrc/cc_host_abi.inc

```

int cc_shard_rows(int32_t n, int32_t world, int32_t rank, int32_t unit, int32_t* lo, int32_t* hi)
{
    if (n < 0 || world < 1 || rank < 0 || rank >= world || unit < 1 || !lo || !hi) return CC_ERR_BAD_ARG;
    int a = 0, b = 0;
    cc_shard_range(n, world, rank, unit, &a, &b);
    *lo = a;
    *hi = b;
    return CC_OK;
}

int64_t cc_format_points_csv(const double* values, int64_t n, int32_t d, int64_t first_id, const int32_t* label_idx,
                             const char* label_bytes, const int32_t* label_offsets, int32_t n_labels, char* out,
                             int64_t cap)
{
    if (!values || n < 0 || d < 0 || !label_idx || !label_bytes || !label_offsets || n_labels < 1 || !out) return CC_ERR_BAD_ARG;
    char* o = out;
    char* const end = out + cap;
    int max_label = 0;
    for (int i = 0; i < n_labels; ++i) max_label = std::max(max_label, label_offsets[i + 1] - label_offsets[i]);
    const int64_t row_max = 24 + 1 + max_label + (int64_t)d * 33 + 2;
    for (int64_t r = 0; r < n; ++r) {
        if (end - o < row_max) return CC_ERR_OOM;
        o += cc::format_i64(first_id + r, o);
        *o++ = ',';
        int li = label_idx[r];
        if (li < 0 || li >= n_labels) li = n_labels - 1;
        const int ll = label_offsets[li + 1] - label_offsets[li];
        memcpy(o, label_bytes + label_offsets[li], (size_t)ll);
        o += ll;
        const double* v = values + r * d;
        for (int i = 0; i < d; ++i) {
            *o++ = ',';
            if (v[i] == v[i]) o += cc::format_repr(v[i], o);
        }
        *o++ = '\n';
    }
    return (int64_t)(o - out);
}

int cc_policy_replay(const cc_policy_config* cfg, cc_policy_carry* carry, int64_t start_cursor, int32_t start_rows,
                     const cc_policy_obs* obs, int32_t n, cc_policy_decision* out)
{
    if (!cfg || !carry || n < 0 || (n > 0 && !obs) || !out) return CC_ERR_BAD_ARG;
    cc::WindowPolicy policy(*cfg, *carry);
    out[0] = policy.start(start_cursor, start_rows);
    for (int i = 0; i < n; ++i)
        out[i + 1] = obs[i].after_sequential ? policy.after_sequential(obs[i].cursor, obs[i].m_rows) : policy.after_batch(obs[i]);
    *carry = policy.carry();
    return CC_OK;
}

double cc_policy_seq_rate_guess(int32_t d, int32_t m_rows, int32_t allow_seq_r, int32_t allow_seq_g)
{
    if (d < 1 || d > CC_MAX_DIM || m_rows < 0) return -1.0;
    const int seq_cap = d > CC_WINDOW_MAX_DIM ? 0 : cc_seq_cap_rows(d);
    return cc::seq_rate_guess(d, m_rows, seq_cap, allow_seq_r != 0, allow_seq_g != 0);
}

int cc_seq_handover_replay(int32_t mode, int32_t possible, int32_t sticky, const cc_seq_event* ev, int32_t n, int32_t* outcome,
                           int64_t* stint_len)
{
    if (mode < 0 || mode > 2 || n < 0 || (n > 0 && !ev) || !outcome || !stint_len) return CC_ERR_BAD_ARG;
    cc::SeqHandover rule;
    outcome[0] = rule.start(mode, possible != 0, sticky != 0) ? 1 : 0;
    stint_len[0] = rule.stint_len();
    for (int i = 0; i < n; ++i) {
        const cc_seq_event& e = ev[i];
        outcome[i + 1] = e.chunk_event
                             ? (int32_t)rule.after_chunk(e.got, e.rate, e.chunk, e.use_g != 0, e.allow_seq_g != 0, e.possible != 0,
                                                         e.more != 0, e.wide != 0)
                             : (rule.after_batch(e.bad != 0, e.rate, e.possible != 0, e.more != 0, e.seq_r_applies != 0, e.rate_guess) ? 1 : 0);
        stint_len[i + 1] = rule.stint_len();
    }
    return CC_OK;
}

int cc_batch_plan(const cc_batch_inputs* in, cc_batch_geometry* out)
{
    if (!in || !out) return CC_ERR_BAD_ARG;
    for (int t : {in->decide_threads, in->chain_threads, in->commit_threads})
        if (t != 64 && t != 128 && t != 256) return CC_ERR_BAD_ARG;
    if (in->window < 1 || in->win_cfg < 0 || in->S_cfg < 1 || in->n_cus < 1 || in->prune_wgs_per_cu < 1 || in->plain_wgs_per_cu < 1 ||
        in->m_rows < 0 || in->long_avg < 0 || in->points_left < 0)
        return CC_ERR_BAD_ARG;
    *out = cc::batch_plan(*in);
    return CC_OK;
}

int cc_scan_width(int32_t d, int32_t filter_on, int32_t k_pow2, int32_t* padded, int32_t* scan_u, int32_t* chain)
{
    if (d < 1 || d > CC_MAX_DIM || !padded || !scan_u || !chain) return CC_ERR_BAD_ARG;
    const cc::ScanWidth w = cc::scan_width(d, filter_on != 0, k_pow2 != 0);
    *padded = w.padded;
    *scan_u = w.scan_u ? 1 : 0;
    *chain = w.chain;
    return CC_OK;
}
```

### chronoclust_amd/csrc/cc_knobs.h

```cpp
#pragma once
#include <algorithm>
#include <climits>
#include <cstdlib>

struct Knobs {
    bool trace = false;
    bool light_sync_events = true;
    int chain_threads = 64, decide_threads = 256, commit_threads = 256;
    int decide_group = 16;
    bool allow_scan_u = true;
    int prune_mode = 1;
    double prune_F = 16.0;
    int prune_rounds4 = 0;
    bool group_guess_always = false;
    bool allow_guess = true;
    bool allow_lean = true;
    int force_prune_rows = 0;
    bool allow_seed16 = false;
    bool allow_prune_general = true;
    bool la_pruned = false;
    bool allow_probe = true;
    int split_a_mode = 1;
    bool allow_nodirty = true;
    bool allow_claims = true;
    bool allow_long = true;
    bool allow_prep = true;
    bool allow_quiet = true;
    bool allow_missed_plain = true;
    int p3_listed_rows = 10000;
    bool allow_scan_p3 = true;
    bool allow_scan_p2 = true;
    bool allow_link = true;
    bool allow_heavy = true;
    bool allow_seq_r = true;
    bool allow_seq_g = true;
    int allow_sparse = 128;
    int assign_chunk = 0;
    int ingest_slab = 0;
    int assign_segments = 0;
};

namespace {

void knob_off_when_starts_with_0(bool& v, const char* name) { const char* e = getenv(name); v = !(e && e[0] == '0'); }
void knob_on_when_starts_with_1(bool& v, const char* name) { const char* e = getenv(name); v = e && e[0] == '1'; }
void knob_atoi_nonzero_when_set(bool& v, const char* name) { if (const char* e = getenv(name)) v = atoi(e) != 0; }
void knob_int_in(int& v, const char* name, int lo, int hi) { const char* e = getenv(name); if (e && atoi(e) >= lo && atoi(e) <= hi) v = atoi(e); }
void knob_threads(int& v, const char* name) { int t = 0; knob_int_in(t, name, 64, 256); if (t == 64 || t == 128 || t == 256) v = t; }

void read_knobs(Knobs& k)
{
    knob_on_when_starts_with_1(k.trace, "CHRONOCLUST_HIP_TRACE");
    knob_on_when_starts_with_1(k.group_guess_always, "CHRONOCLUST_HIP_GROUP_GUESS");
    knob_off_when_starts_with_0(k.allow_nodirty, "CHRONOCLUST_HIP_NODIRTY");
    knob_off_when_starts_with_0(k.allow_claims, "CHRONOCLUST_HIP_CLAIMS");
    knob_off_when_starts_with_0(k.allow_long, "CHRONOCLUST_HIP_LONGCHAINS");
    knob_off_when_starts_with_0(k.allow_prep, "CHRONOCLUST_HIP_LONGPREP");
    knob_off_when_starts_with_0(k.allow_quiet, "CHRONOCLUST_HIP_QUIET");
    knob_off_when_starts_with_0(k.allow_heavy, "CHRONOCLUST_HIP_HEAVY");
    knob_off_when_starts_with_0(k.allow_seq_r, "CHRONOCLUST_HIP_SEQR");
    knob_off_when_starts_with_0(k.allow_seq_g, "CHRONOCLUST_HIP_SEQG");
    knob_off_when_starts_with_0(k.allow_probe, "CHRONOCLUST_HIP_PROBE");
    knob_off_when_starts_with_0(k.allow_guess, "CHRONOCLUST_HIP_GUESS");
    knob_off_when_starts_with_0(k.allow_lean, "CHRONOCLUST_HIP_LEAN");
    knob_off_when_starts_with_0(k.allow_scan_p2, "CHRONOCLUST_HIP_SCANP2");
    knob_off_when_starts_with_0(k.allow_link, "CHRONOCLUST_HIP_LINK");
    knob_atoi_nonzero_when_set(k.light_sync_events, "CHRONOCLUST_HIP_LIGHT_EVENTS");
    knob_atoi_nonzero_when_set(k.allow_scan_u, "CHRONOCLUST_HIP_SCANU");
    knob_atoi_nonzero_when_set(k.allow_seed16, "CHRONOCLUST_HIP_SEED16");
    knob_atoi_nonzero_when_set(k.allow_missed_plain, "CHRONOCLUST_HIP_MISSED_PLAIN");
    knob_atoi_nonzero_when_set(k.allow_prune_general, "CHRONOCLUST_HIP_PRUNE_GENERAL");
    knob_atoi_nonzero_when_set(k.allow_scan_p3, "CHRONOCLUST_HIP_SCANP3");
    knob_atoi_nonzero_when_set(k.la_pruned, "CHRONOCLUST_HIP_LA_PRUNED");
    knob_threads(k.chain_threads, "CHRONOCLUST_HIP_CHAIN_THREADS");
    knob_threads(k.decide_threads, "CHRONOCLUST_HIP_DECIDE_THREADS");
    knob_threads(k.commit_threads, "CHRONOCLUST_HIP_COMMIT_THREADS");
    { int g = 0; knob_int_in(g, "CHRONOCLUST_HIP_DECIDE_GROUP", 16, 32); if (g == 16 || g == 32) k.decide_group = g; }
    knob_int_in(k.prune_mode, "CHRONOCLUST_HIP_PRUNE", 0, 2);
    knob_int_in(k.prune_rounds4, "CHRONOCLUST_HIP_PRUNE_WGS", 1, 64);
    knob_int_in(k.allow_sparse, "CHRONOCLUST_HIP_SPARSE", 0, INT_MAX);
    knob_int_in(k.assign_chunk, "CHRONOCLUST_HIP_ASSIGN_CHUNK", 1, 1 << 24);
    knob_int_in(k.ingest_slab, "CHRONOCLUST_HIP_INGEST_SLAB", 1, 1 << 26);
    knob_int_in(k.assign_segments, "CHRONOCLUST_HIP_ASSIGN_SEGMENTS", 1, 64);
    knob_int_in(k.force_prune_rows, "CHRONOCLUST_HIP_FORCE_PRUNE_ROWS", INT_MIN, INT_MAX);
    knob_int_in(k.p3_listed_rows, "CHRONOCLUST_HIP_P3_LISTED", INT_MIN, INT_MAX);
    if (const char* e = getenv("CHRONOCLUST_HIP_SCANA")) k.split_a_mode = std::max(0, std::min(2, atoi(e)));
    if (const char* e = getenv("CHRONOCLUST_HIP_PRUNE_F")) if (atof(e) >= 1.0) k.prune_F = atof(e);
}

}
```

### chronoclust_amd/csrc/cc_offline.h

```cpp
#pragma once
#include "cc_common.h"


__global__ void k_decay(Table tab, int m_rows, int d, double f)
{
    const int e = blockIdx.x * blockDim.x + threadIdx.x;
    if (e < m_rows * d) {
        tab.cf1[e] = tab.cf1[e] * f;
        tab.cf2[e] = tab.cf2[e] * f;
    }
    if (e < m_rows) tab.w[e] = tab.w[e] * f;
}

__global__ void k_downgrade_flags(Table tab, int m_rows, int d, double beta_mu, int pi, double omicron, int* flags)
{
    const int r = blockIdx.x * blockDim.x + threadIdx.x;
    if (r >= m_rows) return;
    int cnt = 0;
    for (int i = 0; i < d; ++i) cnt += (tab.pref[(size_t)r * d + i] > 1.0);
    const double w = tab.w[r];
    flags[r] = ((w < beta_mu || cnt > pi) ? 1 : 0) | ((w <= omicron) ? 2 : 0);
}

__global__ __launch_bounds__(256) void k_rebuild_scl(Ctl* __restrict__ ctl, Table tab, int m_rows, int d, int pow2, double inv_k)
// ... 118 lines not shown
#pragma unroll
            for (int i = 0; i < DP; ++i) {
                double t = cq[i] - s_p[m * DP + i];
                t = t * t;
                acc = acc + t;
            }
            const bool in = qvalid && sqrt(acc) <= eps;
            const unsigned long long mask = __builtin_amdgcn_ballot_w64(in);
            if (lane == 0) adj[(size_t)(pt + m) * words + qword] = mask;
        }
    }
}

#define CC_EPS_BD 32

__global__ __launch_bounds__(256) void k_eps_neighbours_blk(const double* __restrict__ cen, int mp, int d, double eps,
                                                            unsigned long long* __restrict__ adj, int words, int p_base,
                                                            int p_end, int pch)
{
    __shared__ __attribute__((aligned(16))) double s_p[CC_EPS_TP * CC_EPS_BD];
    const int lane = threadIdx.x & 63, wv = threadIdx.x >> 6;
    const int qword = blockIdx.x * 4 + wv;
    const int q = qword * 64 + lane;
    const bool qvalid = qword < words && q < mp;
    const int p0 = p_base + blockIdx.y * pch;
    const int p1 = min(p_end, p0 + pch);
    for (int pt = p0; pt < p1; pt += CC_EPS_TP) {
        const int tp = min(CC_EPS_TP, p1 - pt);
        double acc[CC_EPS_TP];
#pragma unroll
        for (int m = 0; m < CC_EPS_TP; ++m) acc[m] = 0.0;
        for (int i0 = 0; i0 < d; i0 += CC_EPS_BD) {
            double cq[CC_EPS_BD];
#pragma unroll
            for (int i = 0; i < CC_EPS_BD; ++i) cq[i] = (qvalid && i0 + i < d) ? cen[(size_t)q * d + i0 + i] : 0.0;
            __syncthreads();
            for (int e = threadIdx.x; e < CC_EPS_TP * CC_EPS_BD; e += 256) {
                const int m = e / CC_EPS_BD, i = e - m * CC_EPS_BD;
                s_p[e] = (m < tp && i0 + i < d) ? cen[(size_t)(pt + m) * d + i0 + i] : 0.0;
            }
            __syncthreads();
            if (qword >= words) continue;
#pragma unroll
            for (int m = 0; m < CC_EPS_TP; ++m) {
#pragma unroll
                for (int i = 0; i < CC_EPS_BD; ++i) {
                    double t = cq[i] - s_p[m * CC_EPS_BD + i];
                    t = t * t;
                    acc[m] = acc[m] + t;
                }
            }
        }
        if (qword >= words) continue;
#pragma unroll
        for (int m = 0; m < CC_EPS_TP; ++m) {
            if (m < tp) {
                const bool in = qvalid && sqrt(acc[m]) <= eps;
                const unsigned long long mask = __builtin_amdgcn_ballot_w64(in);
                if (lane == 0) adj[(size_t)(pt + m) * words + qword] = mask;
            }
        }
    }
}

__global__ void k_subspace_pref(const double* __restrict__ cen, const unsigned long long* __restrict__ adj,
                                int words, int mp, int d, double delta, double k, double* __restrict__ wvec,
                                int* __restrict__ nn, int p_base, int p_end)
{
    const int e = p_base * d + blockIdx.x * blockDim.x + threadIdx.x;
    if (e >= p_end * d) return;
    const int p = e / d, c = e - p * d;
    const double cp = cen[e];
    double acc = 0.0;
    int n = 0;
    for (int wd = 0; wd < words; ++wd) {
        unsigned long long m = adj[(size_t)p * words + wd];
        while (m) {
            const int b = __builtin_ctzll(m);
            m &= m - 1;
            const int q = wd * 64 + b;
            double t = cp - cen[(size_t)q * d + c];
            t = t * t;
            acc = acc + t;
            ++n;
        }
    }
    const double var = acc / (double)n;
    wvec[e] = (var <= delta) ? k : 1.0;
    if (c == 0) nn[p] = n;
}

__global__ void k_pdim(const double* __restrict__ wvec, int mp, int d, int* __restrict__ pdim)
{
    const int p = blockIdx.x * blockDim.x + threadIdx.x;
    if (p >= mp) return;
    int cnt = 0;
    for (int i = 0; i < d; ++i) cnt += (wvec[(size_t)p * d + i] > 1.0);
    pdim[p] = cnt;
}

__global__ __launch_bounds__(64) void k_weighted_reach(const double* __restrict__ cen, const double* __restrict__ wvec,
                                                       const unsigned long long* __restrict__ adj,
                                                       unsigned long long* __restrict__ adjw, int words, int mp,
                                                       int d, double eps_sq, int p_base, int p_end)
{
    const int p = p_base + blockIdx.x;
    if (p >= p_end) return;
    const int lane = threadIdx.x;
    for (int w0 = 0; w0 < words; w0 += 64) {
        const int wd = w0 + lane;
        const unsigned long long nb = (wd < words) ? adj[(size_t)p * words + wd] : 0ull;
        unsigned long long res = 0ull;
        for (unsigned long long todo = __builtin_amdgcn_ballot_w64(nb != 0ull); todo; todo &= todo - 1ull) {
            const int l = __builtin_ctzll(todo);
            const unsigned lo = (unsigned)__builtin_amdgcn_readlane((int)(unsigned)(nb & 0xFFFFFFFFull), l);
            const unsigned hi = (unsigned)__builtin_amdgcn_readlane((int)(unsigned)(nb >> 32), l);
            const unsigned long long bits = ((unsigned long long)hi << 32) | lo;
            const int q = (w0 + l) * 64 + lane;
            bool in = false;
            if (q < mp && ((bits >> lane) & 1ull)) {
                double dpq = 0.0, dqp = 0.0;
                for (int i = 0; i < d; ++i) {
                    const double a = cen[(size_t)p * d + i], b = cen[(size_t)q * d + i];
                    double t = a - b;
                    t = t * t;
                    t = wvec[(size_t)p * d + i] * t;
                    dpq = dpq + t;
                    double u = b - a;
                    u = u * u;
                    u = wvec[(size_t)q * d + i] * u;
                    dqp = dqp + u;
                }
                const double dist = dpq > dqp ? dpq : dqp;
                in = dist <= eps_sq;
            }
            const unsigned long long mask = __builtin_amdgcn_ballot_w64(in);
            if (lane == l) res = mask;
        }
        if (wd < words) adjw[(size_t)p * words + wd] = res;
    }
}

__global__ __launch_bounds__(64) void k_adj_counts(const unsigned long long* __restrict__ adjw, int words, int mp,
                                                   int* __restrict__ cnt)
{
    const int p = blockIdx.x;
    if (p >= mp) return;
    int c = 0;
    for (int wd = threadIdx.x; wd < words; wd += 64) c += __builtin_popcountll(adjw[(size_t)p * words + wd]);
    for (int off = 32; off >= 1; off >>= 1) c += __shfl_xor(c, off);
    if (threadIdx.x == 0) cnt[p] = c;
}

__global__ __launch_bounds__(64) void k_adj_fill(const unsigned long long* __restrict__ adjw, int words, int mp,
                                                 const long long* __restrict__ off, int* __restrict__ nbr)
{
    const int p = blockIdx.x;
    if (p >= mp) return;
    const int lane = threadIdx.x;
    long long base = off[p];
    for (int w0 = 0; w0 < words; w0 += 64) {
        const int wd = w0 + lane;
        unsigned long long m = (wd < words) ? adjw[(size_t)p * words + wd] : 0ull;
        const int mine = __builtin_popcountll(m);
        int incl = mine;
        for (int o = 1; o < 64; o <<= 1) {
            const int v = __shfl_up(incl, o);
            if (lane >= o) incl += v;
        }
        long long pos = base + incl - mine;
        while (m) {
            nbr[pos++] = wd * 64 + __builtin_ctzll(m);
            m &= m - 1ull;
        }
        base += __shfl(incl, 63);
    }
}

__global__ void k_cluster_merge(PcoreView pv, const int* __restrict__ members, const int* __restrict__ off, int nc,
                                int d, double delta_sq, double k, double* __restrict__ ccf1, double* __restrict__ ccf2,
                                double* __restrict__ ccen, double* __restrict__ cpref, double* __restrict__ cw)
{
    const int e = blockIdx.x * blockDim.x + threadIdx.x;
    if (e >= nc * d) return;
    const int c = e / d, i = e - c * d;
    double s1 = 0.0, s2 = 0.0, w = 0.0;
    for (int t = off[c]; t < off[c + 1]; ++t) {
        const int m = members[t];
        s1 = s1 + pv.cf1[(size_t)m * d + i];
        s2 = s2 + pv.cf2[(size_t)m * d + i];
        w = w + pv.w[m];
    }
    ccf1[e] = s1;
    ccf2[e] = s2;
    ccen[e] = s1 / w;
    double a = s2 / w;
    double b = s1 / w;
    b = b * b;
    const double var = a - b;
    cpref[e] = (var <= delta_sq) ? k : 1.0;
    if (i == 0) cw[c] = w;
}


#define CC_ASSOC_TQ 32

template <int DP, bool UNIT>
__global__ __launch_bounds__(256) void k_assoc_tiled(const double* __restrict__ cur_cen, const double* __restrict__ cur_op,
                                                     const double* __restrict__ prev_cen, int mc, int mp, int d, int c_lo,
                                                     int c_hi, double* __restrict__ part_dist, int* __restrict__ part_idx)
{
    __shared__ __attribute__((aligned(16))) double s_q[CC_ASSOC_TQ * DP];
    const int lane = threadIdx.x & 63, wv = threadIdx.x >> 6;
    const int c = c_lo + (blockIdx.x * 4 + wv) * 64 + lane;
    const bool valid = c < c_hi;
    double cc[DP], op[DP];
#pragma unroll
    for (int i = 0; i < DP; ++i) {
        cc[i] = (valid && i < d) ? cur_cen[(size_t)c * d + i] : 0.0;
        op[i] = (valid && i < d) ? cur_op[(size_t)c * d + i] : 1.0;
    }
    const int S = gridDim.y;
    const int per = (mp + S - 1) / S;
    const int q0 = blockIdx.y * per, q1 = min(mp, q0 + per);
    double best = __builtin_huge_val();
    int bidx = -1;
    for (int qt = q0; qt < q1; qt += CC_ASSOC_TQ) {
        const int tq = min(CC_ASSOC_TQ, q1 - qt);
        __syncthreads();
        for (int e = threadIdx.x; e < CC_ASSOC_TQ * DP; e += 256) {
            const int m = e / DP, i = e - m * DP;
            s_q[e] = (m < tq && i < d) ? prev_cen[(size_t)(qt + m) * d + i] : 0.0;
        }
        __syncthreads();
        for (int m = 0; m < tq; ++m) {
            double acc = 0.0;
#pragma unroll
            for (int i = 0; i < DP; ++i) {
                double t = s_q[m * DP + i] - cc[i];
                t = t * t;
                t = UNIT ? t * op[i] : ((op[i] != 1.0) ? t / op[i] : t);
                acc = acc + t;
            }
            if (bidx < 0 || acc < best) {
                best = acc;
                bidx = qt + m;
            }
        }
    }
    if (valid) {
        part_dist[(size_t)blockIdx.y * mc + c] = best;
        part_idx[(size_t)blockIdx.y * mc + c] = bidx;
    }
}

#define CC_ASSOC_BD 16

template <bool UNIT>
__global__ __launch_bounds__(256) void k_assoc_tiled_blk(const double* __restrict__ cur_cen, const double* __restrict__ cur_op,
                                                         const double* __restrict__ prev_cen, int mc, int mp, int d, int c_lo,
                                                         int c_hi, double* __restrict__ part_dist, int* __restrict__ part_idx)
{
    __shared__ __attribute__((aligned(16))) double s_q[CC_ASSOC_TQ * CC_ASSOC_BD];
    const int lane = threadIdx.x & 63, wv = threadIdx.x >> 6;
    const int c = c_lo + (blockIdx.x * 4 + wv) * 64 + lane;
    const bool valid = c < c_hi;
    const int S = gridDim.y;
    const int per = (mp + S - 1) / S;
    const int q0 = blockIdx.y * per, q1 = min(mp, q0 + per);
    double best = __builtin_huge_val();
    int bidx = -1;
    for (int qt = q0; qt < q1; qt += CC_ASSOC_TQ) {
        const int tq = min(CC_ASSOC_TQ, q1 - qt);
        double acc[CC_ASSOC_TQ];
#pragma unroll
        for (int m = 0; m < CC_ASSOC_TQ; ++m) acc[m] = 0.0;
        for (int i0 = 0; i0 < d; i0 += CC_ASSOC_BD) {
            double cc[CC_ASSOC_BD], op[CC_ASSOC_BD];
#pragma unroll
            for (int i = 0; i < CC_ASSOC_BD; ++i) {
                cc[i] = (valid && i0 + i < d) ? cur_cen[(size_t)c * d + i0 + i] : 0.0;
                op[i] = (valid && i0 + i < d) ? cur_op[(size_t)c * d + i0 + i] : 1.0;
            }
            __syncthreads();
            for (int e = threadIdx.x; e < CC_ASSOC_TQ * CC_ASSOC_BD; e += 256) {
                const int m = e / CC_ASSOC_BD, i = e - m * CC_ASSOC_BD;
                s_q[e] = (m < tq && i0 + i < d) ? prev_cen[(size_t)(qt + m) * d + i0 + i] : 0.0;
            }
            __syncthreads();
#pragma unroll
            for (int m = 0; m < CC_ASSOC_TQ; ++m) {
#pragma unroll
                for (int i = 0; i < CC_ASSOC_BD; ++i) {
                    double t = s_q[m * CC_ASSOC_BD + i] - cc[i];
                    t = t * t;
                    t = UNIT ? t * op[i] : ((op[i] != 1.0) ? t / op[i] : t);
                    acc[m] = acc[m] + t;
                }
            }
        }
#pragma unroll
        for (int m = 0; m < CC_ASSOC_TQ; ++m) {
            if (m < tq && (bidx < 0 || acc[m] < best)) {
                best = acc[m];
                bidx = qt + m;
            }
        }
    }
    if (valid) {
        part_dist[(size_t)blockIdx.y * mc + c] = best;
        part_idx[(size_t)blockIdx.y * mc + c] = bidx;
    }
}

__global__ void k_assoc_merge(const double* __restrict__ part_dist, const int* __restrict__ part_idx, int S, int mc,
                              int c_lo, int c_hi, int* __restrict__ out_idx, double* __restrict__ out_dist)
{
    const int c = c_lo + blockIdx.x * blockDim.x + threadIdx.x;
    if (c >= c_hi) return;
    double best = __builtin_huge_val();
    int bidx = -1;
    for (int s = 0; s < S; ++s) {
        const int i = part_idx[(size_t)s * mc + c];
        const double v = part_dist[(size_t)s * mc + c];
        if (i >= 0 && (bidx < 0 || v < best)) {
            best = v;
            bidx = i;
        }
// ... 14 lines not shown
```

### chronoclust_amd/csrc/cc_online_run.h

```cpp
#pragma once

namespace {

struct PolicyTrace {
    FILE* f = nullptr;
    static void obs_json(FILE* f, const cc_policy_obs& o)
    {
        fprintf(f, "{\"cursor\": %lld, \"m_rows\": %d, \"stall_b\": %d, \"stat_windows\": %lld, \"stat_truncated\": %lld, "
                   "\"stat_trunc_unknown\": %lld, \"stat_tiles\": %lld, \"stat_dirty_tiles\": %lld, \"stat_unsafe\": %lld, \"stat_missed\": %lld, \"tg_ok\": %d, \"round_hist\": [",
                (long long)o.cursor, o.m_rows, o.stall_b, (long long)o.stat_windows, (long long)o.stat_truncated,
                (long long)o.stat_trunc_unknown, (long long)o.stat_tiles, (long long)o.stat_dirty_tiles, (long long)o.stat_unsafe,
                (long long)o.stat_missed, o.tg_ok);
        for (int r = 0; r < CC_POLICY_MAX_ROUNDS + 2; ++r) fprintf(f, "%s%lld", r ? ", " : "", (long long)o.round_hist[r]);
        fprintf(f, "], \"prune_rows\": %llu, \"prune_full\": %llu, \"after_sequential\": %d}", (unsigned long long)o.prune_rows,
                (unsigned long long)o.prune_full, o.after_sequential);
    }
    static void dec_json(FILE* f, const cc_policy_decision& d)
    {
        fprintf(f, "{\"win_cfg\": %d, \"want\": %d, \"rounds\": %d, \"batch_windows\": %d, \"lookahead\": %d, \"nodirty\": %d, "
                   "\"prune\": %d, \"shard\": %d, \"restart\": %d, \"bad\": %d, \"stalled\": %d, \"sparse\": %d, \"probe\": %d}",
                d.win_cfg, d.want, d.rounds, d.batch_windows, d.lookahead, d.nodirty, d.prune, d.shard, d.restart, d.bad, d.stalled, d.sparse, d.probe);
    }
    PolicyTrace(const cc_policy_config& c, const cc_policy_carry& k, long long cursor, int rows, const cc_policy_decision& d0,
                int rank)
// ... 115 lines not shown
    c.n_heavy = c.n_heavy_new = 0;
    c.stat_seq_clk = c.stat_seq_wall = 0;
    c.stat_prune_rows = c.stat_prune_full = 0;
    c.stat_missed = 0;
    c.seed_at = -1;
    for (int q = 0; q < 2; ++q) {
        c.n_missed[q] = 0;
        for (int K = 0; K < 2; ++K) { c.tg[q][K] = 0.0; c.tg_ok[q][K] = 0; }
    }
    c.cen_absmax = 0ull;
    c.stat_pair_rows = 0.0;
    for (int i = 0; i < CC_MAX_ROUNDS + 2; ++i) c.round_hist[i] = 0;
}

struct OnlineRun {
    cc_handle* const h;
    const long long range_a, N;
    const bool no_create, resume;
    Ctl& c;

    int win = 0, R = 0;
    int S_cfg = 1, Sd_full = 1, Sd = 1;
    int world = 1, myrank = 0;
    bool grouped = false;
    size_t batch_max = 2;
    bool timing = false;
    int seq_cap = 0;
    Versions ver{};
    Carry car{};
    hipStream_t sA = nullptr, sB = nullptr;
    static constexpr size_t ev_base = 4;

    std::optional<cc::WindowPolicy> policy;
    std::optional<PolicyTrace> ptrace;
    cc_policy_decision dec{};
    bool nodirty = false;
    bool sparse_now = false;
    bool la_on = false;
    bool shard_on = false;
    bool link_now = false;
    int Rcur = 1;
    int batch_windows = 2;

    long long done = 0;
    int m_known = 0;
    unsigned long long seq_host = 0;
    long long cursor_prev = 0;
    double batch_t0 = 0.0;

    hipEvent_t ev0 = nullptr, ev1 = nullptr, evCommit = nullptr, evScan = nullptr;
    size_t ev_used = 2, ev_sync = ev_base;
    std::vector<std::pair<size_t, double>> timed;
    std::vector<size_t> timed_comm;
    double pair_rows_eff = 0.0, pair_rows_prev = 0.0;
    double pair_rows_pruned = 0.0;
    long long sharded_windows = 0;

    cc::SeqHandover seq;
    cc::LongChains longs;
    long long long_launches = 0;

    cc::BatchPlan bp{};
    Table tab{};
    Rows trows{}, vrows{}, crows{}, vrows_sp{}, crows_sp{}, srows[2] = {};
    ScanCopy scopy[2] = {};
    int* long_list = nullptr;
    int probe_left = 0;
    hipEvent_t scan_end = nullptr;

    OnlineRun(cc_handle* handle, long long a, long long e, bool no_create_, bool resume_)
        : h(handle), range_a(a), N(e), no_create(no_create_), resume(resume_), c(handle->hc) {}

    static double now_ms()
    {
        return std::chrono::duration<double, std::milli>(std::chrono::steady_clock::now().time_since_epoch()).count();
    }
    bool seq_r_applies() const { return h->allow_seq_r && h->d >= 2 && h->d <= 4; }
    bool wide() const { return h->d > CC_WINDOW_MAX_DIM; }
    size_t window_rows() const { return wide() ? 0 : (size_t)win * batch_max; }
    bool seq_g_applies() const { return h->allow_seq_g && h->hc.m_rows >= seq_cap; }
    double seq_rate_guess() const { return cc::seq_rate_guess(h->d, h->hc.m_rows, seq_cap, h->allow_seq_r, h->allow_seq_g); }
    bool seq_possible() const { return !h->comm.active() && !no_create && (h->hc.m_rows < seq_cap || h->allow_seq_g); }

    void set_lookahead(bool on)
    {
        la_on = on;
        c.la_on = on ? 1 : 0;
        c.stall_b = 0;
        c.mode = 0;
        c.car_n = 0;
        const int q = (int)((c.window_seq + 1ull) & 1ull);
        const long long c1 = c.cursor + c.win_b;
        const long long left1 = c.n_points - c1;
        c.la_cursor[q] = c1;
        c.la_b[q] = (on && left1 > 0) ? (int)std::min<long long>(left1, c.win_cfg) : 0;
        c.la_rows[q] = c.m_rows;
        c.la_cursor[q ^ 1] = 0;
        c.la_b[q ^ 1] = 0;
        c.la_rows[q ^ 1] = 0;
    }

    cc_policy_config policy_config() const
    {
        const ScanPlan& plan = h->scan_plan;
        cc_policy_config p{};
        p.window = win; p.rounds_max = R; p.n_end = N; p.d = h->d; p.resume = resume ? 1 : 0;
        p.windows_per_sync = h->tun.windows_per_sync; p.early_window = h->tun.early_window; p.lookahead = h->tun.lookahead;
        p.allow_nodirty = h->allow_nodirty ? 1 : 0; p.allow_sparse = h->allow_sparse; p.lookahead_pruned = h->la_pruned ? 1 : 0;
        p.prune_mode = h->prune_mode; p.prune_applicable = plan.prune_applicable; p.force_prune_rows = plan.force_prune_rows;
        p.allow_guess = plan.allow_guess; p.allow_probe = plan.allow_probe;
        p.can_shard = (grouped && !h->shard_suspended) ? 1 : 0;
        p.shard_min_row_dims = h->shard_min_row_dims; p.shard_min_row_dims_pruned = h->shard_min_row_dims_pruned;
        return p;
    }

    void prepare()
    {
        refresh_ctl_params(h);
        h->scan_plan = scan_plan(h);
        const ScanPlan& plan = h->scan_plan;
        win = h->tun.window; R = h->tun.rounds;
        S_cfg = std::max(1, h->tun.segments / plan.waves);
        Sd_full = std::max(1, (h->tun.dirty_segments > 0 ? h->tun.dirty_segments : h->tun.segments) / plan.dirty_waves);
        Sd = Sd_full;
        nodirty = false;
        ensure_window_buffers(h, wide() ? 64 : win, std::max(S_cfg, Sd_full));
        world = h->comm.world; myrank = h->comm.rank;
        grouped = h->comm.active();
        if (grouped) {
            const size_t gmax = (size_t)std::max(64, h->win_alloc);
            h->gsend_stride = gmax * 4 + 4;
            h->gpart_stride = (size_t)world * (gmax * 4 + 4);
            h->gsend.ensure(2 * h->gsend_stride);
            h->gpart.ensure(2 * h->gpart_stride);
            h->gsend2.ensure((size_t)2 * CC_MISSED_CAP * 4);
            h->gpart2.ensure((size_t)2 * world * CC_MISSED_CAP * 4);
        }
        batch_max = (size_t)std::max(2, h->tun.windows_per_sync);
        ensure_table(h, (size_t)h->hc.m_rows + window_rows() + 1);

        c.cursor = range_a;
        c.n_points = N;
        c.xt_stride = h->n_points;
        c.no_create = no_create ? 1 : 0;
        const cc_policy_config pcfg = policy_config();
        const cc_policy_carry pcarry{h->adapt_win, h->clean_batches, h->since_shrink, 0};
        policy.emplace(pcfg, pcarry);
        dec = policy->start(range_a, c.m_rows);
        ptrace.emplace(pcfg, pcarry, range_a, c.m_rows, dec, grouped ? myrank : -1);
        c.win_cfg = dec.win_cfg;
        c.win_b = (int)std::min<long long>(c.win_cfg, N - range_a);
        c.max_rounds = R;
        reset_call_counters(c);
        HIPCHK(hipMemsetAsync(h->tab.heavy.p, 0, h->tab.cap * sizeof(int), h->stream));
        c.x_absmax = h->x_absmax;
        set_lookahead(dec.lookahead != 0);
        push_ctl(h);

        HIPCHK(hipMemsetAsync(h->rec.p, 0, sizeof(CommitRec), h->stream));
        HIPCHK(hipMemsetAsync(h->cmax.p, 0, 2 * sizeof(unsigned long long), h->stream));
        HIPCHK(hipMemsetAsync(h->found.p, 0, h->found.n * sizeof(unsigned long long), h->stream));
        HIPCHK(hipMemsetAsync(h->lstat.p, 0, h->lstat.n * sizeof(unsigned long long), h->stream));
        HIPCHK(hipMemsetAsync(h->lprev.p, 0, h->lprev.n * sizeof(unsigned long long), h->stream));
        if (c.m_rows > 0)
            hipLaunchKernelGGL(k_rebuild_scl, dim3((c.m_rows * h->d + 255) / 256), dim3(256), 0, h->stream, h->ctl.p, h->tab.view(),
                               c.m_rows, h->d, c.pow2, c.inv_k);
        ev0 = get_event(h, 0); ev1 = get_event(h, 1);
        HIPCHK(hipEventRecord(ev0, h->stream));
        ev_used = 2;
        timing = h->tun.time_kernels != 0;
        shard_on = dec.shard != 0;

        ver = versions_view(h);
        car = carry_view(h);
        sA = h->stream; sB = h->stream2;
        evCommit = get_event(h, 2); evScan = nullptr;
        ev_sync = ev_base;
        ev_used = ev_base + 3 * (batch_max + 2);

        done = range_a;
        m_known = c.m_rows;
        seq_cap = wide() ? 0 : cc_seq_cap_rows(h->d);
        seq.start(wide() ? 2 : h->tun.sequential, seq_possible(), h->seq_sticky);
        Rcur = dec.rounds;
        batch_windows = dec.batch_windows;
        h->set_prune(dec.prune);
        nodirty = dec.nodirty != 0;
        sparse_now = dec.sparse != 0;
        cursor_prev = range_a;
        seq_host = c.window_seq;
        link_now = h->allow_link && !no_create && !wide();
    }

    void sequential_stint()
    {
        const int chunk = 8192;
        const double t0 = now_ms();
        const bool use_g = seq_g_applies();
        const bool f = h->hc.filter != 0, p2 = h->hc.pow2 != 0;
        if (use_g) {
            const int list_cap = (int)std::min<size_t>(h->tab.cap, (size_t)INT_MAX / 2);
            h->seq_lists.ensure(2 * (size_t)list_cap);
            h->seq_img.ensure(4 * (size_t)list_cap * (size_t)h->d);
            with_bools([&](auto F, auto P, auto W) {
                hipLaunchKernelGGL((k_seq_g<decltype(F)::value, decltype(P)::value, decltype(W)::value>), dim3(1), dim3(CC_SEQG_THREADS), 0, sA, h->ctl.p, h->X.p, tab,
                                   h->lab_uid.p, h->lab_path.p, chunk, h->seq_lists.p, list_cap, h->seq_img.p);
            }, f, p2, h->d > CC_SEQG_NARROW_DIM);
        } else {
            int follow = 0;
            auto seq_r = [&](auto D) {
                with_bools([&](auto P) {
                    hipLaunchKernelGGL((k_seq_r<decltype(D)::value, decltype(P)::value>), dim3(1), dim3(64), 0, sA, h->ctl.p, h->X.p, tab, h->lab_uid.p,
                                       h->lab_path.p, chunk);
                }, p2);
                follow = 1;
            };
            if (h->allow_seq_r) {
                if (h->d == 2) seq_r(std::integral_constant<int, 2>{});
                else if (h->d == 3) seq_r(std::integral_constant<int, 3>{});
                else if (h->d == 4) seq_r(std::integral_constant<int, 4>{});
            }
            with_bools([&](auto F, auto P) {
                hipLaunchKernelGGL((k_seq<decltype(F)::value, decltype(P)::value>), dim3(1), dim3(64), 0, sA, h->ctl.p, h->X.p, tab, h->lab_uid.p,
                                   h->lab_path.p, chunk, follow);
            }, f, p2);
        }
        HIPCHK(hipGetLastError());
        pull_ctl(h);
        const double dt = now_ms() - t0;
        const long long got = h->hc.cursor - done;
        done = h->hc.cursor;
        m_known = h->hc.m_rows;
        seq_host = h->hc.window_seq;
        cursor_prev = h->hc.cursor;
        const double seq_rate = got > 0 ? (double)got / std::max(dt, 1e-3) : 0.0;
        if (h->trace)
            fprintf(stderr, "[cc] done %lld rows %d | sequential kernel: %lld points in %.3f ms (so far %lld shader cycles, %.3f ms of kernel time)\n",
                    done, h->hc.m_rows, got, dt, (long long)h->hc.stat_seq_clk, (double)h->hc.stat_seq_wall / 1e5);
        if (use_g) h->stats.seq_g_points += got;
        if (seq.after_chunk(got, seq_rate, chunk, use_g, h->allow_seq_g, seq_possible(), done < N, wide()) != cc::SeqHandover::kContinue) {
            HIPCHK(hipMemsetAsync(h->rec.p, 0, sizeof(CommitRec), h->stream));
            h->hc.win_b = (int)std::min<long long>(h->hc.win_cfg, N - done);
            dec = policy->after_sequential(h->hc.cursor, h->hc.m_rows);
            ptrace->sequential(h->hc.cursor, h->hc.m_rows, dec);
            nodirty = dec.nodirty != 0;
            sparse_now = dec.sparse != 0;
            set_lookahead(dec.lookahead != 0);
            push_ctl(h);
        }
    }

    cc::BatchInputs batch_inputs() const
    {
        const ScanPlan& plan = h->scan_plan;
        cc::BatchInputs in{};
        in.window = win; in.win_cfg = h->hc.win_cfg; in.batch_windows = batch_windows; in.points_left = N - done;
        in.S_cfg = S_cfg; in.n_cus = h->n_cus; in.prune_wgs_per_cu = plan.prune_wgs_per_cu; in.plain_wgs_per_cu = plan.plain_wgs_per_cu;
        in.prune_now = h->prune_now ? 1 : 0;
        in.decide_threads = h->decide_threads; in.chain_threads = h->chain_threads; in.commit_threads = h->commit_threads;
        in.allow_claims = h->allow_claims ? 1 : 0; in.allow_long = h->allow_long ? 1 : 0;
        in.allow_heavy = h->allow_heavy ? 1 : 0; in.allow_prep = h->allow_prep ? 1 : 0;
        in.m_rows = h->hc.m_rows; in.n_heavy = h->hc.n_heavy;
        in.long_seen = longs.seen ? 1 : 0; in.long_few = longs.few ? 1 : 0; in.long_avg = longs.avg;
        return in;
    }


    int* claims_of(int round) const { return (round & 1) ? h->T1.p : h->T0.p; }
    const ScanCopy& sc_now() const { return scopy[seq_host & 1ull]; }
    int quiet_ok() const { return h->allow_quiet ? 1 : 0; }
    bool sparse_round() const { return nodirty && sparse_now; }

    void exchange_missed(hipStream_t st, const Rows& rws, int mode, int round, int q, int srank, int sworld)
    {
        launch_scan<false>(h, st, bp.gw, rws, nullptr, h->part.p, bp.S, round, mode, srank, sworld, 1);
        Cand* const send2 = h->gsend2.p + (size_t)q * CC_MISSED_CAP * 4;
        Cand* const recv2 = h->gpart2.p + (size_t)q * sworld * CC_MISSED_CAP * 4;
        hipLaunchKernelGGL(k_merge_partials, dim3((CC_MISSED_CAP + 255) / 256), dim3(256), 0, st, h->ctl.p,
                           h->part.p, h->part_stride, bp.S, send2, (size_t)0, round, mode,
                           (const unsigned long long*)nullptr, 0, (const int*)h->missed.p);
        h->comm.all_gather(send2, recv2, (size_t)CC_MISSED_CAP * 4 * sizeof(Cand), st, st == h->stream2 ? 1 : 0);
        hipLaunchKernelGGL(k_scatter_missed, dim3((CC_MISSED_CAP * sworld + 255) / 256), dim3(256), 0, st,
                           (const Ctl*)h->ctl.p, (const int*)h->missed.p, (const Cand*)recv2, sworld,
                           h->gpart.p, h->gpart_stride, (size_t)bp.gw * 4 + 4, round, mode);
    }

    void snapshot_scan(hipStream_t st, int mode, int round)
    {
        const int gw = bp.gw, S = bp.S;
        const int q = (mode == 1) ? (round & 1) : (int)(seq_host & 1ull);
        const Rows& src = (mode == 1) ? srows[round & 1] : trows;
        const Rows rws = h->scan_plan.pad_rows ? padded_rows(h, st, src, q, round, mode) : src;
        h->probe_now = probe_left > 0 && !h->prune_now;
        if (h->probe_now) --probe_left;
        const int srank = shard_on ? myrank : 0, sworld = shard_on ? world : 1;
        h->group_guess_now = shard_on && (sworld > 1 || h->group_guess_always);
        scan_end = nullptr;
        if (timing) {
            hipEvent_t a = get_event(h, ev_used), b = get_event(h, ev_used + 1);
            HIPCHK(hipEventRecord(a, st));
            launch_scan<false>(h, st, gw, rws, nullptr, h->part.p, S, round, mode, srank, sworld);
            HIPCHK(hipEventRecord(b, st));
            timed.push_back({ev_used, h->prune_now ? 1.0 : 0.0});
            ev_used += 2;
            if (!shard_on) scan_end = b;
        } else {
            launch_scan<false>(h, st, gw, rws, nullptr, h->part.p, S, round, mode, srank, sworld);
        }
        if (!shard_on) return;
        if (timing) HIPCHK(hipEventRecord(get_event(h, ev_used), st));
        hipLaunchKernelGGL(k_merge_partials, dim3((gw + 255) / 256), dim3(256), 0, st, h->ctl.p, h->part.p,
                           h->part_stride, S, h->gsend.p, h->gsend_stride, round, mode,
                           (const unsigned long long*)h->pstat_p(), gw * 4,
                           (const int*)nullptr);
        h->comm.all_gather(h->gsend.p + (size_t)q * h->gsend_stride, h->gpart.p + (size_t)q * h->gpart_stride,
                           ((size_t)gw * 4 + 4) * sizeof(Cand), st, st == h->stream2 ? 1 : 0);
// ... 330 lines not shown
```

### include/chronoclust_hip.h

```cpp
#ifndef CHRONOCLUST_HIP_H
#define CHRONOCLUST_HIP_H

#include <stdint.h>

#ifdef __cplusplus
extern "C" {
#endif

typedef struct cc_handle cc_handle;

enum cc_status {
    CC_OK = 0,
    CC_ERR_NO_DEVICE = -1,
    CC_ERR_BAD_ARG = -2,
    CC_ERR_NONFINITE = -3,
    CC_ERR_OOM = -4,
    CC_ERR_INTERNAL = -5,
    CC_ERR_COMM = -6
};

enum cc_kind { CC_PCORE = 0, CC_OUTLIER = 1 };

#define CC_MAX_DIM 1024
#define CC_WINDOW_MAX_DIM 64
// ... 57 lines not shown
    int64_t probe_launches;
    int64_t seq_r_points;
    int64_t heavy_launches;
    int64_t scan_lean_launches;
    int64_t long_prepared;
    int64_t long_replayed;
    int64_t seq_g_points;
    int64_t link_launches;
    int64_t scan_p2_launches;
    double  calib_allgather_us;
    double  calib_scan_ns_per_row_dim;
    int64_t split_threshold_row_dims;
    int64_t split_threshold_row_dims_pruned;
    int64_t missed_plain_launches;
    int64_t seed16_launches;
    int64_t pad_rows_launches;
    int64_t assign_points;
    int64_t assign_launches;
} cc_stats;

int cc_create(int device, cc_handle** out);
void cc_destroy(cc_handle* h);
const char* cc_last_error(const cc_handle* h);
int cc_set_tuning(cc_handle* h, const cc_tuning* t);
int cc_reset(cc_handle* h);

int cc_set_params(cc_handle* h, const cc_params* p);

int cc_decay_downgrade(cc_handle* h, double factor);

int cc_points_upload(cc_handle* h, const double* x, int64_t n, int32_t d);
int cc_points_prefetch(cc_handle* h, const double* x, int64_t n, int32_t d, const double* scale, const double* min_);
int cc_online_run(cc_handle* h);
int cc_labels_download(cc_handle* h, int64_t* out_uid, int8_t* out_path);
int cc_online(cc_handle* h, const double* x, int64_t n, int32_t d, int64_t* out_uid, int8_t* out_path);

int cc_assign(cc_handle* h, const double* x, int64_t n, int32_t d, int64_t* out_uid, int8_t* out_path, double* out_dist);

int cc_points_upload_f32(cc_handle* h, const float* x, int64_t n, int32_t d);
int cc_points_upload_scaled_f32(cc_handle* h, const float* x, int64_t n, int32_t d, const double* scale,
                                const double* min_);
int cc_points_prefetch_f32(cc_handle* h, const float* x, int64_t n, int32_t d, const double* scale, const double* min_);
int cc_col_minmax_f32(cc_handle* h, const float* x, int64_t n, int32_t d, double* out_min, double* out_max);
int cc_online_f32(cc_handle* h, const float* x, int64_t n, int32_t d, int64_t* out_uid, int8_t* out_path);
int cc_assign_f32(cc_handle* h, const float* x, int64_t n, int32_t d, int64_t* out_uid, int8_t* out_path, double* out_dist);
int cc_points_download_xt(cc_handle* h, double* out);
int cc_f32_points(cc_handle* h, int64_t* out);

enum cc_dtype {
    CC_DT_F64 = 0, CC_DT_F32 = 1, CC_DT_F16 = 2,
    CC_DT_I8 = 3, CC_DT_U8 = 4, CC_DT_I16 = 5, CC_DT_U16 = 6, CC_DT_I32 = 7, CC_DT_U32 = 8
};

typedef struct cc_points_view {
    const void* data;
    int64_t n;
    int32_t d;
    int32_t dtype;
    int64_t row_stride;
    int64_t col_stride;
} cc_points_view;

int cc_points_upload_view(cc_handle* h, const cc_points_view* view, const double* scale, const double* min_);
int cc_points_prefetch_view(cc_handle* h, const cc_points_view* view, const double* scale, const double* min_);
int cc_col_minmax_view(cc_handle* h, const cc_points_view* view, double* out_min, double* out_max);
int cc_online_view(cc_handle* h, const cc_points_view* view, int64_t* out_uid, int8_t* out_path);
int cc_assign_view(cc_handle* h, const cc_points_view* view, int64_t* out_uid, int8_t* out_path, double* out_dist);
int cc_view_points(cc_handle* h, int64_t* out);

#define CC_MAX_SRC_COLS 4096
enum { CC_LM_SWAPPED = 1 };
typedef struct cc_list_mode {
    const void* data;
    int64_t n;
    int32_t src_cols;
    int32_t dtype;
    int32_t flags;
    int32_t d;
    const int32_t* cols;
    const uint32_t* masks;
} cc_list_mode;

int cc_points_upload_list(cc_handle* h, const cc_list_mode* lm, const double* scale, const double* min_);
int cc_points_prefetch_list(cc_handle* h, const cc_list_mode* lm, const double* scale, const double* min_);
int cc_col_minmax_list(cc_handle* h, const cc_list_mode* lm, double* out_min, double* out_max);
int cc_online_list(cc_handle* h, const cc_list_mode* lm, int64_t* out_uid, int8_t* out_path);
int cc_assign_list(cc_handle* h, const cc_list_mode* lm, int64_t* out_uid, int8_t* out_path, double* out_dist);
int cc_list_points(cc_handle* h, int64_t* out);

#define CC_MAX_COMP 64
typedef struct cc_list_transform {
    int32_t m;
    int32_t reserved;
    const int32_t* comp_cols;
    const double* comp;
    const double* cofactor;
} cc_list_transform;
int cc_points_upload_list_xf(cc_handle* h, const cc_list_mode* lm, const cc_list_transform* xf, const double* scale,
                             const double* min_);
int cc_points_prefetch_list_xf(cc_handle* h, const cc_list_mode* lm, const cc_list_transform* xf, const double* scale,
                               const double* min_);
int cc_col_minmax_list_xf(cc_handle* h, const cc_list_mode* lm, const cc_list_transform* xf, double* out_min, double* out_max);
int cc_online_list_xf(cc_handle* h, const cc_list_mode* lm, const cc_list_transform* xf, int64_t* out_uid, int8_t* out_path);
int cc_assign_list_xf(cc_handle* h, const cc_list_mode* lm, const cc_list_transform* xf, int64_t* out_uid, int8_t* out_path,
                      double* out_dist);

int cc_count(cc_handle* h, int kind);
int cc_dim(cc_handle* h);
int cc_counters(cc_handle* h, int64_t* pcore_last_id, int64_t* outlier_last_id);
int cc_set_counters(cc_handle* h, int64_t pcore_last_id, int64_t outlier_last_id);
int cc_export(cc_handle* h, int kind, int64_t* id, int64_t* uid, double* w,
              double* cf1, double* cf2, double* cen, double* pref);
int cc_inject_mc(cc_handle* h, int kind, int32_t d, const double* cf1, const double* cf2, const double* cen,
                 const double* pref, double w, int64_t id, int64_t uid);

int cc_inject_bulk(cc_handle* h, int kind, int32_t d, int32_t n, const double* cf1, const double* cf2,
                   const double* cen, const double* pref, const double* w, const int64_t* id, const int64_t* uid);

int cc_offline(cc_handle* h, int32_t* n_clusters, int8_t* out_core, int32_t* out_pdim, int32_t* out_nn,
               int32_t* out_nw);
int cc_num_core(cc_handle* h);
int cc_cluster_size(cc_handle* h, int32_t c);
int cc_cluster_export(cc_handle* h, int32_t c, int64_t* members, double* w, double* cf1, double* cf2,
                      double* cen, double* pref);

int cc_clusters_total_members(cc_handle* h);
int cc_clusters_export(cc_handle* h, int64_t* members, int32_t* offsets, double* w, double* cf1, double* cf2,
                       double* cen, double* pref);

int cc_col_minmax(cc_handle* h, const double* x, int64_t n, int32_t d, double* out_min, double* out_max);
int cc_points_upload_scaled(cc_handle* h, const double* x, int64_t n, int32_t d, const double* scale,
                            const double* min_);
int cc_points_download(cc_handle* h, double* out, const double* scale, const double* min_);

int cc_assoc_argmin(cc_handle* h, const double* cur_cen, const double* cur_pref, int32_t mc,
                    const double* prev_cen, int32_t mp, int32_t d, int32_t* out_idx, double* out_dist);

#define CC_COMM_ID_BYTES 128
int cc_comm_unique_id(void* out_id);
int cc_comm_init_rccl(cc_handle* h, const void* id_bytes, int rank, int world);
int cc_comm_init_local(cc_handle** handles, int world);
int cc_comm_calibrate(cc_handle* h);
int cc_comm_destroy(cc_handle* h);
int cc_comm_info(cc_handle* h, int32_t* rank, int32_t* world, int32_t* transport);
int cc_comm_set_relaxed(cc_handle* h, int32_t minibatch_points);
typedef struct cc_relaxed_stats {
    int64_t super_steps;
    int64_t minibatch_points;
    int64_t deferred_points;
    int64_t reserved[5];
} cc_relaxed_stats;
int cc_get_relaxed_stats(cc_handle* h, cc_relaxed_stats* out);
int cc_shard_rows(int32_t n, int32_t world, int32_t rank, int32_t unit, int32_t* lo, int32_t* hi);
int cc_set_shard_thresholds(cc_handle* h, int64_t min_row_dims, int32_t offline_min_rows);

int cc_point_clusters(cc_handle* h, int32_t* out_idx);

int64_t cc_format_points_csv(const double* values, int64_t n, int32_t d, int64_t first_id, const int32_t* label_idx,
                             const char* label_bytes, const int32_t* label_offsets, int32_t n_labels, char* out,
                             int64_t cap);

int cc_sync(cc_handle* h);

int cc_get_stats(cc_handle* h, cc_stats* out);

#define CC_POLICY_MAX_ROUNDS 8
typedef struct cc_policy_config {
    int32_t window, rounds_max, windows_per_sync, early_window;
    int32_t lookahead;
    int32_t allow_nodirty;
    int32_t prune_mode;
    int32_t prune_applicable;
    int32_t can_shard;
    int32_t d;
    int32_t resume;
    int32_t allow_sparse;
    int32_t allow_guess;
    int32_t allow_probe;
    int64_t shard_min_row_dims;
    int64_t n_end;
    int64_t shard_min_row_dims_pruned;
    int32_t lookahead_pruned;
    int32_t force_prune_rows;
} cc_policy_config;
typedef struct cc_policy_carry {
    int32_t adapt_win, clean_batches, since_shrink, pad;
} cc_policy_carry;
typedef struct cc_policy_obs {
    int64_t cursor;
    int32_t m_rows, stall_b;
    int64_t stat_windows, stat_truncated, stat_trunc_unknown, stat_tiles, stat_dirty_tiles;
    int64_t stat_unsafe;
    int64_t stat_missed;
    int64_t round_hist[CC_POLICY_MAX_ROUNDS + 2];
    uint64_t prune_rows, prune_full;
    int32_t after_sequential;
    int32_t tg_ok;
} cc_policy_obs;
typedef struct cc_policy_decision {
    int32_t win_cfg;
    int32_t want;
    int32_t rounds, batch_windows, lookahead, nodirty;
    int32_t prune;
    int32_t shard;
    int32_t restart;
    int32_t bad;
    int32_t stalled;
    int32_t sparse;
    int32_t probe;
    int32_t pad;
    int64_t wins, pts, trunc, unk, tiles, dtiles, grew, prune_rows, prune_full;
} cc_policy_decision;
int cc_policy_replay(const cc_policy_config* cfg, cc_policy_carry* carry, int64_t start_cursor, int32_t start_rows,
                     const cc_policy_obs* obs, int32_t n, cc_policy_decision* out);
double cc_policy_seq_rate_guess(int32_t d, int32_t m_rows, int32_t allow_seq_r, int32_t allow_seq_g);
typedef struct cc_seq_event {
    int32_t chunk_event;
    int32_t bad;
    int32_t possible;
    int32_t more;
    int32_t seq_r_applies;
    int32_t use_g;
    int32_t allow_seq_g, wide;
    int64_t got, chunk;
    double rate;
    double rate_guess;
} cc_seq_event;
int cc_seq_handover_replay(int32_t mode, int32_t possible, int32_t sticky, const cc_seq_event* ev, int32_t n, int32_t* outcome,
                           int64_t* stint_len);

typedef struct cc_batch_inputs {
    int32_t window, win_cfg;
    int32_t S_cfg;
    int32_t n_cus, prune_now;
    int32_t prune_wgs_per_cu, plain_wgs_per_cu;
    int32_t decide_threads, chain_threads, commit_threads;
    int32_t allow_claims, allow_long, allow_heavy, allow_prep;
    int32_t m_rows, n_heavy;
    int32_t long_seen, long_few;
    int64_t long_avg;
    int32_t batch_windows, pad;
    int64_t points_left;
} cc_batch_inputs;
enum { CC_LONG_NONE = 0, CC_LONG_ROWS_SPLIT = 1, CC_LONG_ROWS_SMALL = 2, CC_LONG_LIST_SPLIT = 3, CC_LONG_LIST_SMALL = 4 };
typedef struct cc_batch_geometry {
    int32_t gw;
    int32_t S;
    int32_t sparse_cap;
    int32_t dblocks, cblocks, rblocks;
    int32_t scan_rows;
    int32_t long_rows;
    int32_t long_listed;
    int32_t heavy_on;
    int32_t long_cap;
    int32_t windows_now;
    int32_t prep;
    int32_t prep_form;
    int32_t long_form;
    int32_t pad;
} cc_batch_geometry;
int cc_batch_plan(const cc_batch_inputs* in, cc_batch_geometry* out);

enum { CC_CHAIN_NONE = 0, CC_CHAIN_COMMON = 1, CC_CHAIN_GENERAL = 2 };
int cc_scan_width(int32_t d, int32_t filter_on, int32_t k_pow2, int32_t* padded, int32_t* scan_u, int32_t* chain);

#ifdef __cplusplus
}
#endif
#endif
```

Measured before the change: 77.96 million points/s.

## Cut offline host round-trips: device scan, packed readback, staged cluster sums, fused clears

Several host-side offline-phase costs are reworked. The std::sort of pcore rows becomes a radix sort. The neighbour-list offset scan moves to a single-block device kernel, and all per-pcore arrays are packed into one block so a speculative neighbour fill and readback happen in one trip. Cluster sums are staged to pinned host memory behind an event so later per-cluster getters avoid separate D2H copies. Six memsets at online-run start are merged into one clearing kernel. The cost is more pinned memory, a possible second fill pass when the edge cap is exceeded, and more complex bookkeeping.

```diff
diff --git a/chronoclust_amd/_lib.py b/chronoclust_amd/_lib.py
--- a/chronoclust_amd/_lib.py
+++ b/chronoclust_amd/_lib.py
@@ -341,6 +341,7 @@
     "cc_scan_width": (C.c_int, [C.c_int32, C.c_int32, C.c_int32, _i32p, _i32p, _i32p]),
     "cc_shard_rows": (C.c_int, [C.c_int32, C.c_int32, C.c_int32, C.c_int32, _i32p, _i32p]),
     "cc_set_shard_thresholds": (C.c_int, [C.c_void_p, C.c_int64, C.c_int32]),
+    "cc_list_order": (C.c_int32, [_i32p, _i32p, C.c_int32, C.c_int32, _i32p]),
 }
 
 COMM_ID_BYTES = 128
@@ -370,7 +371,7 @@
 
 
 HOST_ONLY_SYMBOLS = ("cc_policy_replay", "cc_policy_seq_rate_guess", "cc_seq_handover_replay", "cc_batch_plan", "cc_shard_rows",
-                     "cc_format_points_csv", "cc_scan_width")
+                     "cc_format_points_csv", "cc_scan_width", "cc_list_order")
 
 
 def load_host_only(path):
@@ -551,6 +552,18 @@
     return lo.value, hi.value
 
 
+def list_order(kind, key, which_kind):
+    kind = np.ascontiguousarray(kind, dtype=np.int32)
+    key = np.ascontiguousarray(key, dtype=np.int32)
+    if kind.shape != key.shape or kind.ndim != 1:
+        raise ValueError("kind and key: two vectors of one length")
+    rows = np.empty(len(kind), np.int32)
+    n = load().cc_list_order(_ptr(kind, _i32p), _ptr(key, _i32p), len(kind), int(which_kind), _ptr(rows, _i32p))
+    if n < 0:
+        raise ValueError("cc_list_order: %s" % _ERRORS.get(n, n))
+    return rows[:n]
+
+
 _DESCRIBED = ("view", "list", "list_xf")
 _INGEST = {
     "upload": {"f64": "cc_points_upload", "f32": "cc_points_upload_f32",
diff --git a/chronoclust_amd/csrc/cc_api.hip b/chronoclust_amd/csrc/cc_api.hip
--- a/chronoclust_amd/csrc/cc_api.hip
+++ b/chronoclust_amd/csrc/cc_api.hip
@@ -388,6 +388,7 @@
     }
     for (hipEvent_t e : h->ev_pool) (void)hipEventDestroy(e);
     for (hipEvent_t e : h->sync_pool) (void)hipEventDestroy(e);
+    if (h->c_stage_ev) (void)hipEventDestroy(h->c_stage_ev);
     delete h;
 }
 
@@ -423,10 +424,12 @@
         h->clean_batches = 0;
         h->since_shrink = 1000;
         h->clusters.clear();
+        h->c_staged = false;
         h->n_core = 0;
         refresh_ctl_params(h);
         push_ctl(h);
         sync_stream(h, h->stream);
+        h->c_stage_pending = false;
         return (int)CC_OK;
     });
 }
diff --git a/chronoclust_amd/csrc/cc_api_offline.inc b/chronoclust_amd/csrc/cc_api_offline.inc
--- a/chronoclust_amd/csrc/cc_api_offline.inc
+++ b/chronoclust_amd/csrc/cc_api_offline.inc
@@ -5,26 +5,27 @@
     std::vector<int> pcore, outlier;
 };
 
-RowList list_order(cc_handle* h, std::vector<int>* kind_out = nullptr, std::vector<int>* key_out = nullptr)
+RowList list_order(cc_handle* h)
 {
     const int m = h->hc.m_rows;
+    RowList rl;
+    if (m == 0) return rl;
     std::vector<int> kind(m), key(m);
-    if (m) {
-        HIPCHK(hipMemcpyAsync(kind.data(), h->tab.kind.p, (size_t)m * 4, hipMemcpyDeviceToHost, h->stream));
-        HIPCHK(hipMemcpyAsync(key.data(), h->tab.key.p, (size_t)m * 4, hipMemcpyDeviceToHost, h->stream));
-        sync_stream(h, h->stream);
-    }
-    RowList rl;
-    for (int r = 0; r < m; ++r) {
-        if (kind[r] == CC_KIND_PCORE) rl.pcore.push_back(r);
-        else if (kind[r] == CC_KIND_OUTLIER) rl.outlier.push_back(r);
-    }
-    auto by_key = [&](int a, int b) { return key[a] < key[b]; };
-    std::sort(rl.pcore.begin(), rl.pcore.end(), by_key);
-    std::sort(rl.outlier.begin(), rl.outlier.end(), by_key);
-    if (kind_out) *kind_out = kind;
-    if (key_out) *key_out = key;
+    HIPCHK(hipMemcpyAsync(kind.data(), h->tab.kind.p, (size_t)m * 4, hipMemcpyDeviceToHost, h->stream));
+    HIPCHK(hipMemcpyAsync(key.data(), h->tab.key.p, (size_t)m * 4, hipMemcpyDeviceToHost, h->stream));
+    sync_stream(h, h->stream);
+    rl.pcore.resize((size_t)m);
+    rl.pcore.resize((size_t)cc_list_order_rows(kind.data(), key.data(), m, CC_KIND_PCORE, rl.pcore.data()));
+    rl.outlier.resize((size_t)m);
+    rl.outlier.resize((size_t)cc_list_order_rows(kind.data(), key.data(), m, CC_KIND_OUTLIER, rl.outlier.data()));
     return rl;
+}
+
+void wait_stage(cc_handle* h)
+{
+    if (!h->c_stage_pending) return;
+    HIPCHK(hipEventSynchronize(h->c_stage_ev));
+    h->c_stage_pending = false;
 }
 
 }
@@ -117,9 +118,13 @@
         auto now_us = []() { return std::chrono::duration<double, std::micro>(std::chrono::steady_clock::now().time_since_epoch()).count(); };
         double tph[8] = {now_us(), 0, 0, 0, 0, 0, 0, 0};
         const int m_all = h->hc.m_rows;
+        wait_stage(h);
+        h->c_staged = false;
         h->pin.reset();
-        h->pin.reserve((size_t)m_all * 72 + ((size_t)1 << 16));
-        std::vector<int> prow_host;
+        const size_t pin_budget = (size_t)m_all * 88 + ((size_t)1 << 16);
+        h->pin.reserve(pin_budget);
+        int mp = 0;
+        const int* prow_pin = nullptr;
         const long long* uid_all = nullptr;
         if (m_all > 0) {
             int* kind = h->pin.take<int>((size_t)m_all);
@@ -130,16 +135,12 @@
             HIPCHK(hipMemcpyAsync(uid, h->tab.uid.p, (size_t)m_all * 8, hipMemcpyDeviceToHost, h->stream));
             sync_stream(h, h->stream);
             uid_all = uid;
-            std::vector<unsigned long long> order;
-            order.reserve((size_t)m_all);
-            for (int r = 0; r < m_all; ++r)
-                if (kind[r] == CC_KIND_PCORE) order.push_back(((unsigned long long)((unsigned)key[r] ^ 0x80000000u) << 32) | (unsigned)r);
-            std::sort(order.begin(), order.end());
-            prow_host.resize(order.size());
-            for (size_t i = 0; i < order.size(); ++i) prow_host[i] = (int)(order[i] & 0xFFFFFFFFull);
+            int* rows = h->pin.take<int>((size_t)m_all);
+            mp = cc_list_order_rows(kind, key, m_all, CC_KIND_PCORE, rows);
+            prow_pin = rows;
         }
         tph[1] = now_us();
-        const int mp = (int)prow_host.size(), d = h->d;
+        const int d = h->d;
         if (mp == 0) return (int)CC_OK;
         const size_t md = (size_t)mp * d;
         const int words = (mp + 63) / 64;
@@ -152,8 +153,6 @@
         h->pv_cf1.ensure(md); h->pv_cf2.ensure(md); h->pv_cen.ensure(md); h->pv_pref.ensure(md); h->pv_w.ensure(mp);
         h->pv_id.ensure(mp); h->prow.ensure(mp); h->wvec.ensure(rows_pad * d); h->nn.ensure(rows_pad); h->pdim.ensure(mp);
         h->core.ensure(mp); h->adj.ensure(rows_pad * words); h->adjw.ensure(rows_pad * words);
-        int* const prow_pin = h->pin.take<int>((size_t)mp);
-        memcpy(prow_pin, prow_host.data(), (size_t)mp * 4);
         HIPCHK(hipMemcpyAsync(h->prow.p, prow_pin, (size_t)mp * 4, hipMemcpyHostToDevice, h->stream));
         PcoreView pv{h->pv_cf1.p, h->pv_cf2.p, h->pv_cen.p, h->pv_pref.p, h->pv_w.p, h->pv_id.p};
         const Ctl& c = h->hc;
@@ -195,36 +194,41 @@
         if (shard)
             h->comm.all_gather(h->adjw.p + (size_t)rank * share * words, h->adjw.p, (size_t)share * words * 8, h->stream);
         h->nw_cnt.ensure(mp);
+        const size_t blk_bytes = OfflineBlock::bytes((size_t)mp);
+        h->host_blk.ensure(blk_bytes);
+        const OfflineBlock blk = OfflineBlock::carve(h->host_blk.p, (size_t)mp);
+        char* const blk_pin = h->pin.take<char>(blk_bytes);
+        const OfflineBlock hb = OfflineBlock::carve(blk_pin, (size_t)mp);
+        const size_t pin_later = (size_t)mp * 8 + 512;
+        const long long cap_room = (long long)((pin_budget - ((h->pin.used + 63) & ~(size_t)63) - pin_later) / 4);
+        const long long cap = h->offline_edge_cap > 0 ? std::min(h->offline_edge_cap, cap_room) : cap_room;
+        h->nw_nbr.ensure((size_t)cap);
+        int* const nbr_pin = h->pin.take<int>((size_t)cap);
         hipLaunchKernelGGL(k_adj_counts, dim3(mp), dim3(64), 0, h->stream, h->adjw.p, words, mp, h->nw_cnt.p);
+        hipLaunchKernelGGL(k_adj_scan, dim3(1), dim3(1024), 0, h->stream, h->nw_cnt.p, h->pv_id.p, h->pdim.p, h->nn.p, h->core.p,
+                           mp, blk);
+        hipLaunchKernelGGL(k_adj_fill, dim3(mp), dim3(64), 0, h->stream, h->adjw.p, words, mp, blk.off, h->nw_nbr.p, cap);
+        HIPCHK(hipMemcpyAsync(blk_pin, h->host_blk.p, blk_bytes, hipMemcpyDeviceToHost, h->stream));
+        HIPCHK(hipMemcpyAsync(nbr_pin, h->nw_nbr.p, (size_t)cap * 4, hipMemcpyDeviceToHost, h->stream));
         h->pcore_uid_host.resize(mp);
-        for (int i = 0; i < mp; ++i) h->pcore_uid_host[(size_t)i] = uid_all[(size_t)prow_host[(size_t)i]];
-        int8_t* const core = h->pin.take<int8_t>((size_t)mp);
-        int* const pdim = h->pin.take<int>((size_t)mp);
-        int* const nn = h->pin.take<int>((size_t)mp);
-        int* const nw_cnt = h->pin.take<int>((size_t)mp);
-        long long* const ids_pin = h->pin.take<long long>((size_t)mp);
-        long long* const nw_off = h->pin.take<long long>((size_t)mp + 1);
-        HIPCHK(hipMemcpyAsync(core, h->core.p, mp, hipMemcpyDeviceToHost, h->stream));
-        HIPCHK(hipMemcpyAsync(pdim, h->pdim.p, (size_t)mp * 4, hipMemcpyDeviceToHost, h->stream));
-        HIPCHK(hipMemcpyAsync(nn, h->nn.p, (size_t)mp * 4, hipMemcpyDeviceToHost, h->stream));
-        HIPCHK(hipMemcpyAsync(nw_cnt, h->nw_cnt.p, (size_t)mp * 4, hipMemcpyDeviceToHost, h->stream));
-        HIPCHK(hipMemcpyAsync(ids_pin, h->pv_id.p, (size_t)mp * 8, hipMemcpyDeviceToHost, h->stream));
+        for (int i = 0; i < mp; ++i) h->pcore_uid_host[(size_t)i] = uid_all[(size_t)prow_pin[(size_t)i]];
         sync_stream(h, h->stream);
         HIPCHK(hipGetLastError());
-        h->pcore_ids_host.assign(ids_pin, ids_pin + mp);
+        const int8_t* const core = hb.core;
+        const int* const pdim = hb.pdim;
+        const int* const nn = hb.nn;
+        const int* const nw_cnt = hb.cnt;
+        const long long* const nw_off = hb.off;
+        h->pcore_ids_host.assign(hb.ids, hb.ids + mp);
         tph[2] = now_us();
-        nw_off[0] = 0;
-        for (int i = 0; i < mp; ++i) nw_off[(size_t)i + 1] = nw_off[i] + nw_cnt[i];
         const long long n_edges = nw_off[mp];
         std::vector<int> nbr_pageable;
-        const int* nbr = nullptr;
-        if (n_edges > 0) {
-            h->nw_off.ensure((size_t)mp + 1);
+        const int* nbr = nbr_pin;
+        if (n_edges > cap) {
             h->nw_nbr.ensure((size_t)n_edges);
-            HIPCHK(hipMemcpyAsync(h->nw_off.p, nw_off, ((size_t)mp + 1) * 8, hipMemcpyHostToDevice, h->stream));
-            hipLaunchKernelGGL(k_adj_fill, dim3(mp), dim3(64), 0, h->stream, h->adjw.p, words, mp, h->nw_off.p, h->nw_nbr.p);
+            hipLaunchKernelGGL(k_adj_fill, dim3(mp), dim3(64), 0, h->stream, h->adjw.p, words, mp, blk.off, h->nw_nbr.p, n_edges);
             int* dst;
-            if (h->pin.used + (size_t)n_edges * 4 + 128 <= h->pin.cap) dst = h->pin.take<int>((size_t)n_edges);
+            if (h->pin.used + (size_t)n_edges * 4 + 128 + pin_later <= h->pin.cap) dst = h->pin.take<int>((size_t)n_edges);
             else {
                 nbr_pageable.resize((size_t)n_edges);
                 dst = nbr_pageable.data();
@@ -271,21 +275,41 @@
         const int nc = (int)h->clusters.size();
         if (nc) {
             const std::vector<int>&mem = h->clusters.mem, &off = h->clusters.off;
-            const size_t cd = (size_t)nc * d;
+            const size_t cd = (size_t)nc * d, c_doubles = (size_t)nc + 4 * cd;
             h->mem_dev.ensure(mem.size()); h->off_dev.ensure(off.size());
-            h->c_cf1.ensure(cd); h->c_cf2.ensure(cd); h->c_cen.ensure(cd); h->c_pref.ensure(cd); h->c_w.ensure(nc);
-            HIPCHK(hipMemcpyAsync(h->mem_dev.p, mem.data(), mem.size() * 4, hipMemcpyHostToDevice, h->stream));
-            HIPCHK(hipMemcpyAsync(h->off_dev.p, off.data(), off.size() * 4, hipMemcpyHostToDevice, h->stream));
+            h->c_blk.ensure(c_doubles);
+            h->c_nc = (size_t)nc;
+            h->c_d = (size_t)d;
+            int* const mem_pin = h->pin.take<int>(mem.size());
+            int* const off_pin = h->pin.take<int>(off.size());
+            memcpy(mem_pin, mem.data(), mem.size() * 4);
+            memcpy(off_pin, off.data(), off.size() * 4);
+            HIPCHK(hipMemcpyAsync(h->mem_dev.p, mem_pin, mem.size() * 4, hipMemcpyHostToDevice, h->stream));
+            HIPCHK(hipMemcpyAsync(h->off_dev.p, off_pin, off.size() * 4, hipMemcpyHostToDevice, h->stream));
             hipLaunchKernelGGL(k_cluster_merge, dim3((unsigned)((cd + 255) / 256)), dim3(256), 0, h->stream, pv,
-                               h->mem_dev.p, h->off_dev.p, nc, d, p.delta_sq, p.k, h->c_cf1.p, h->c_cf2.p, h->c_cen.p,
-                               h->c_pref.p, h->c_w.p);
-            sync_stream(h, h->stream);
+                               h->mem_dev.p, h->off_dev.p, nc, d, p.delta_sq, p.k, h->c_part(1), h->c_part(2), h->c_part(3),
+                               h->c_part(4), h->c_part(0));
+            const bool stage = h->offline_stage && c_doubles * 8 <= ((size_t)16 << 20);
+            if (stage) {
+                h->c_stage.reset();
+                h->c_stage.reserve(c_doubles * 8);
+                HIPCHK(hipMemcpyAsync(h->c_stage.take<double>(c_doubles), h->c_blk.p, c_doubles * 8, hipMemcpyDeviceToHost, h->stream));
+                if (!h->c_stage_ev) HIPCHK(hipEventCreateWithFlags(&h->c_stage_ev, hipEventDisableTiming));
+            }
+            if (stage && !(h->comm.rccl() || h->comm.broken)) {
+                HIPCHK(hipEventRecord(h->c_stage_ev, h->stream));
+                h->c_stage_pending = true;
+            } else {
+                sync_stream(h, h->stream);
+            }
+            h->c_staged = stage;
         }
         tph[5] = now_us();
         if (h->trace)
             fprintf(stderr, "[cc] offline phase, host wall time: list order %.0f us, pair kernels + read-back %.0f, neighbour lists %.0f, "
-                    "ordered expansion %.0f, cluster sums %.0f (%d pcores, %d clusters)\n", tph[1] - tph[0], tph[2] - tph[1], tph[3] - tph[2],
-                    tph[4] - tph[3], tph[5] - tph[4], mp, nc);
+                    "ordered expansion %.0f, cluster sums %.0f (%d pcores, %lld list entries of %lld read in the first trip, %d clusters%s)\n",
+                    tph[1] - tph[0], tph[2] - tph[1], tph[3] - tph[2], tph[4] - tph[3], tph[5] - tph[4], mp, n_edges, cap, nc,
+                    h->c_stage_pending ? ", their sums on their way" : "");
         if (out_core) memcpy(out_core, core, mp);
         if (out_pdim) memcpy(out_pdim, pdim, (size_t)mp * 4);
         if (out_nn) memcpy(out_nn, nn, (size_t)mp * 4);
@@ -308,15 +332,22 @@
 {
     if (!h || c < 0 || c >= (int)h->clusters.size()) return CC_ERR_BAD_ARG;
     return guarded(h, [&]() {
-        const size_t d = (size_t)h->d;
+        const size_t d = h->c_d;
         const int a = h->clusters.off[(size_t)c], e = h->clusters.off[(size_t)c + 1];
         if (members)
             for (int i = a; i < e; ++i) members[i - a] = h->pcore_ids_host[(size_t)h->clusters.mem[(size_t)i]];
-        if (w) HIPCHK(hipMemcpyAsync(w, h->c_w.p + c, 8, hipMemcpyDeviceToHost, h->stream));
-        if (cf1) HIPCHK(hipMemcpyAsync(cf1, h->c_cf1.p + (size_t)c * d, d * 8, hipMemcpyDeviceToHost, h->stream));
-        if (cf2) HIPCHK(hipMemcpyAsync(cf2, h->c_cf2.p + (size_t)c * d, d * 8, hipMemcpyDeviceToHost, h->stream));
-        if (cen) HIPCHK(hipMemcpyAsync(cen, h->c_cen.p + (size_t)c * d, d * 8, hipMemcpyDeviceToHost, h->stream));
-        if (pref) HIPCHK(hipMemcpyAsync(pref, h->c_pref.p + (size_t)c * d, d * 8, hipMemcpyDeviceToHost, h->stream));
+        const double* const src[5] = {w ? h->c_part(0) + c : nullptr, cf1 ? h->c_part(1) + (size_t)c * d : nullptr,
+                                      cf2 ? h->c_part(2) + (size_t)c * d : nullptr, cen ? h->c_part(3) + (size_t)c * d : nullptr,
+                                      pref ? h->c_part(4) + (size_t)c * d : nullptr};
+        double* const dst[5] = {w, cf1, cf2, cen, pref};
+        if (h->c_staged) {
+            wait_stage(h);
+            for (int i = 0; i < 5; ++i)
+                if (dst[i]) memcpy(dst[i], (const double*)h->c_stage.p + (src[i] - h->c_blk.p), (i ? d : 1) * 8);
+            return (int)CC_OK;
+        }
+        for (int i = 0; i < 5; ++i)
+            if (dst[i]) HIPCHK(hipMemcpyAsync(dst[i], src[i], (i ? d : 1) * 8, hipMemcpyDeviceToHost, h->stream));
         sync_stream(h, h->stream);
         return (int)CC_OK;
     });
@@ -335,18 +366,25 @@
 {
     if (!h) return CC_ERR_BAD_ARG;
     return guarded(h, [&]() {
-        const size_t nc = h->clusters.size(), d = (size_t)h->d;
+        const size_t nc = h->clusters.size(), d = h->c_d;
         const size_t tot = h->clusters.mem.size();
         if (offsets)
             for (size_t c = 0; c <= nc; ++c) offsets[c] = (int32_t)h->clusters.off[c];
         if (members)
             for (size_t i = 0; i < tot; ++i) members[i] = h->pcore_ids_host[(size_t)h->clusters.mem[i]];
         if (nc == 0) return (int)CC_OK;
-        if (w) HIPCHK(hipMemcpyAsync(w, h->c_w.p, nc * 8, hipMemcpyDeviceToHost, h->stream));
-        if (cf1) HIPCHK(hipMemcpyAsync(cf1, h->c_cf1.p, nc * d * 8, hipMemcpyDeviceToHost, h->stream));
-        if (cf2) HIPCHK(hipMemcpyAsync(cf2, h->c_cf2.p, nc * d * 8, hipMemcpyDeviceToHost, h->stream));
-        if (cen) HIPCHK(hipMemcpyAsync(cen, h->c_cen.p, nc * d * 8, hipMemcpyDeviceToHost, h->stream));
-        if (pref) HIPCHK(hipMemcpyAsync(pref, h->c_pref.p, nc * d * 8, hipMemcpyDeviceToHost, h->stream));
+        double* const dst[5] = {w, cf1, cf2, cen, pref};
+        if (h->c_staged) {
+            const double t0 = h->trace ? std::chrono::duration<double, std::micro>(std::chrono::steady_clock::now().time_since_epoch()).count() : 0.0;
+            wait_stage(h);
+            const double t1 = h->trace ? std::chrono::duration<double, std::micro>(std::chrono::steady_clock::now().time_since_epoch()).count() : 0.0;
+            for (int i = 0; i < 5; ++i)
+                if (dst[i]) memcpy(dst[i], (const double*)h->c_stage.p + (h->c_part(i) - h->c_blk.p), (i ? nc * d : nc) * 8);
+            if (h->trace) fprintf(stderr, "[cc] clusters export: waited %.0f us for the cluster sums\n", t1 - t0);
+            return (int)CC_OK;
+        }
+        for (int i = 0; i < 5; ++i)
+            if (dst[i]) HIPCHK(hipMemcpyAsync(dst[i], h->c_part(i), (i ? nc * d : nc) * 8, hipMemcpyDeviceToHost, h->stream));
         sync_stream(h, h->stream);
         return (int)CC_OK;
     });
diff --git a/chronoclust_amd/csrc/cc_handle.h b/chronoclust_amd/csrc/cc_handle.h
--- a/chronoclust_amd/csrc/cc_handle.h
+++ b/chronoclust_amd/csrc/cc_handle.h
@@ -200,10 +200,15 @@
     DevBuf<double> pv_cf1, pv_cf2, pv_cen, pv_pref, pv_w, wvec;
     DevBuf<long long> pv_id;
     DevBuf<int> prow, nn, pdim, mem_dev, off_dev, nw_cnt, nw_nbr;
-    DevBuf<long long> nw_off;
+    DevBuf<char> host_blk;
     DevBuf<int8_t> core;
     DevBuf<unsigned long long> adj, adjw;
-    DevBuf<double> c_cf1, c_cf2, c_cen, c_pref, c_w;
+    DevBuf<double> c_blk;
+    size_t c_nc = 0, c_d = 0;
+    double* c_part(int which) const { return c_blk.p + (which == 0 ? 0 : c_nc + (size_t)(which - 1) * c_nc * c_d); }
+    PinArena c_stage;
+    hipEvent_t c_stage_ev = nullptr;
+    bool c_staged = false, c_stage_pending = false;
     HostClusters clusters;
     PinArena pin;
     std::vector<long long> pcore_ids_host, pcore_uid_host;
diff --git a/chronoclust_amd/csrc/cc_host.h b/chronoclust_amd/csrc/cc_host.h
--- a/chronoclust_amd/csrc/cc_host.h
+++ b/chronoclust_amd/csrc/cc_host.h
@@ -1,5 +1,7 @@
 #pragma once
 #include <stdint.h>
+#include <string.h>
+#include <vector>
 
 #if defined(__HIPCC__) || defined(__HIP__)
 #define CC_HOSTDEV __host__ __device__
@@ -24,3 +26,44 @@
 
 #define CC_SEQ_DOUBLES 6600
 CC_HOSTDEV inline int cc_seq_cap_rows(int d) { return CC_SEQ_DOUBLES / (4 * d + 5); }
+
+inline int cc_list_order_rows(const int32_t* kind, const int32_t* key, int m, int which_kind, int32_t* rows_out)
+{
+    int n = 0;
+    bool ascending = true;
+    uint32_t prev = 0;
+    for (int r = 0; r < m; ++r) {
+        if (kind[r] != which_kind) continue;
+        const uint32_t u = (uint32_t)key[r] ^ 0x80000000u;
+        ascending = ascending && (n == 0 || prev <= u);
+        prev = u;
+        rows_out[n++] = r;
+    }
+    if (ascending || n < 2) return n;
+    std::vector<uint64_t> a((size_t)n), b((size_t)n);
+    std::vector<uint32_t> hist((size_t)4 * 256, 0u);
+    for (int i = 0; i < n; ++i) {
+        const uint32_t u = (uint32_t)key[rows_out[i]] ^ 0x80000000u;
+        a[(size_t)i] = ((uint64_t)u << 32) | (uint32_t)rows_out[i];
+        for (int pass = 0; pass < 4; ++pass) ++hist[(size_t)pass * 256 + ((u >> (8 * pass)) & 255u)];
+    }
+    uint64_t* src = a.data();
+    uint64_t* dst = b.data();
+    for (int pass = 0; pass < 4; ++pass) {
+        uint32_t* hp = hist.data() + (size_t)pass * 256;
+        const int shift = 32 + 8 * pass;
+        if (hp[(src[0] >> shift) & 255u] == (uint32_t)n) continue;
+        uint32_t sum = 0;
+        for (int v = 0; v < 256; ++v) {
+            const uint32_t c = hp[v];
+            hp[v] = sum;
+            sum += c;
+        }
+        for (int i = 0; i < n; ++i) dst[hp[(src[i] >> shift) & 255u]++] = src[i];
+        uint64_t* t = src;
+        src = dst;
+        dst = t;
+    }
+    for (int i = 0; i < n; ++i) rows_out[i] = (int32_t)(src[i] & 0xFFFFFFFFull);
+    return n;
+}
diff --git a/chronoclust_amd/csrc/cc_host_abi.inc b/chronoclust_amd/csrc/cc_host_abi.inc
--- a/chronoclust_amd/csrc/cc_host_abi.inc
+++ b/chronoclust_amd/csrc/cc_host_abi.inc
@@ -7,6 +7,12 @@
     *lo = a;
     *hi = b;
     return CC_OK;
+}
+
+int32_t cc_list_order(const int32_t* kind, const int32_t* key, int32_t m, int32_t which_kind, int32_t* rows_out)
+{
+    if (m < 0 || (m > 0 && (!kind || !key || !rows_out))) return CC_ERR_BAD_ARG;
+    return cc_list_order_rows(kind, key, m, which_kind, rows_out);
 }
 
 int64_t cc_format_points_csv(const double* values, int64_t n, int32_t d, int64_t first_id, const int32_t* label_idx,
diff --git a/chronoclust_amd/csrc/cc_knobs.h b/chronoclust_amd/csrc/cc_knobs.h
--- a/chronoclust_amd/csrc/cc_knobs.h
+++ b/chronoclust_amd/csrc/cc_knobs.h
@@ -37,6 +37,8 @@
     int allow_sparse = 128;
     int assign_chunk = 0;
     int ingest_slab = 0;
+    long long offline_edge_cap = 0;
+    bool offline_stage = true;
     int assign_segments = 0;
 };
 
@@ -81,6 +83,8 @@
     knob_int_in(k.allow_sparse, "CHRONOCLUST_HIP_SPARSE", 0, INT_MAX);
     knob_int_in(k.assign_chunk, "CHRONOCLUST_HIP_ASSIGN_CHUNK", 1, 1 << 24);
     knob_int_in(k.ingest_slab, "CHRONOCLUST_HIP_INGEST_SLAB", 1, 1 << 26);
+    knob_off_when_starts_with_0(k.offline_stage, "CHRONOCLUST_HIP_OFFLINE_STAGE");
+    if (const char* e = getenv("CHRONOCLUST_HIP_OFFLINE_EDGE_CAP")) k.offline_edge_cap = std::max(0ll, atoll(e));
     knob_int_in(k.assign_segments, "CHRONOCLUST_HIP_ASSIGN_SEGMENTS", 1, 64);
     knob_int_in(k.force_prune_rows, "CHRONOCLUST_HIP_FORCE_PRUNE_ROWS", INT_MIN, INT_MAX);
     knob_int_in(k.p3_listed_rows, "CHRONOCLUST_HIP_P3_LISTED", INT_MIN, INT_MAX);
diff --git a/chronoclust_amd/csrc/cc_offline.h b/chronoclust_amd/csrc/cc_offline.h
--- a/chronoclust_amd/csrc/cc_offline.h
+++ b/chronoclust_amd/csrc/cc_offline.h
@@ -294,8 +294,66 @@
     if (threadIdx.x == 0) cnt[p] = c;
 }
 
+struct OfflineBlock {
+    long long* off;
+    long long* ids;
+    int* pdim;
+    int* nn;
+    int* cnt;
+    int8_t* core;
+    static __host__ __device__ size_t bytes(size_t mp) { return (mp + 1) * 8 + mp * 8 + 3 * mp * 4 + mp; }
+    static __host__ __device__ OfflineBlock carve(void* base, size_t mp)
+    {
+        OfflineBlock b;
+        b.off = (long long*)base;
+        b.ids = b.off + mp + 1;
+        b.pdim = (int*)(b.ids + mp);
+        b.nn = b.pdim + mp;
+        b.cnt = b.nn + mp;
+        b.core = (int8_t*)(b.cnt + mp);
+        return b;
+    }
+};
+
+__global__ __launch_bounds__(1024) void k_adj_scan(const int* __restrict__ cnt, const long long* __restrict__ ids,
+                                                   const int* __restrict__ pdim, const int* __restrict__ nn,
+                                                   const int8_t* __restrict__ core, int mp, OfflineBlock out)
+{
+    __shared__ long long wave_sum[16];
+    const int lane = threadIdx.x & 63, wave = threadIdx.x >> 6;
+    long long base = 0;
+    for (int t0 = 0; t0 < mp; t0 += 1024) {
+        const int i = t0 + (int)threadIdx.x;
+        const int c = i < mp ? cnt[i] : 0;
+        if (i < mp) {
+            out.ids[i] = ids[i];
+            out.pdim[i] = pdim[i];
+            out.nn[i] = nn[i];
+            out.cnt[i] = c;
+            out.core[i] = core[i];
+        }
+        long long incl = c;
+        for (int o = 1; o < 64; o <<= 1) {
+            const long long v = __shfl_up(incl, o);
+            if (lane >= o) incl += v;
+        }
+        if (lane == 63) wave_sum[wave] = incl;
+        __syncthreads();
+        long long before = 0, tile = 0;
+        for (int w = 0; w < 16; ++w) {
+            const long long v = wave_sum[w];
+            if (w < wave) before += v;
+            tile += v;
+        }
+        if (i < mp) out.off[i] = base + before + incl - c;
+        base += tile;
+        __syncthreads();
+    }
+    if (threadIdx.x == 0) out.off[mp] = base;
+}
+
 __global__ __launch_bounds__(64) void k_adj_fill(const unsigned long long* __restrict__ adjw, int words, int mp,
-                                                 const long long* __restrict__ off, int* __restrict__ nbr)
+                                                 const long long* __restrict__ off, int* __restrict__ nbr, long long cap)
 {
     const int p = blockIdx.x;
     if (p >= mp) return;
@@ -312,10 +370,36 @@
         }
         long long pos = base + incl - mine;
         while (m) {
-            nbr[pos++] = wd * 64 + __builtin_ctzll(m);
+            if (pos < cap) nbr[pos] = wd * 64 + __builtin_ctzll(m);
+            ++pos;
             m &= m - 1ull;
         }
         base += __shfl(incl, 63);
+    }
+}
+
+#define CC_CLEAR_MAX 6
+struct ClearList {
+    unsigned* p[CC_CLEAR_MAX];
+    unsigned long long words[CC_CLEAR_MAX];
+};
+__global__ __launch_bounds__(256) void k_clear_regions(ClearList cl)
+{
+    unsigned long long total = 0;
+#pragma unroll
+    for (int r = 0; r < CC_CLEAR_MAX; ++r) total += cl.words[r];
+    const unsigned long long stride = (unsigned long long)gridDim.x * blockDim.x;
+    for (unsigned long long i = (unsigned long long)blockIdx.x * blockDim.x + threadIdx.x; i < total; i += stride) {
+        unsigned long long j = i;
+        unsigned* at = nullptr;
+#pragma unroll
+        for (int r = 0; r < CC_CLEAR_MAX; ++r) {
+            if (at == nullptr) {
+                if (j < cl.words[r]) at = cl.p[r] + j;
+                else j -= cl.words[r];
+            }
+        }
+        if (at) *at = 0u;
     }
 }
 
diff --git a/chronoclust_amd/csrc/cc_online_run.h b/chronoclust_amd/csrc/cc_online_run.h
--- a/chronoclust_amd/csrc/cc_online_run.h
+++ b/chronoclust_amd/csrc/cc_online_run.h
@@ -291,16 +291,20 @@
         c.win_b = (int)std::min<long long>(c.win_cfg, N - range_a);
         c.max_rounds = R;
         reset_call_counters(c);
-        HIPCHK(hipMemsetAsync(h->tab.heavy.p, 0, h->tab.cap * sizeof(int), h->stream));
         c.x_absmax = h->x_absmax;
         set_lookahead(dec.lookahead != 0);
         push_ctl(h);
 
-        HIPCHK(hipMemsetAsync(h->rec.p, 0, sizeof(CommitRec), h->stream));
-        HIPCHK(hipMemsetAsync(h->cmax.p, 0, 2 * sizeof(unsigned long long), h->stream));
-        HIPCHK(hipMemsetAsync(h->found.p, 0, h->found.n * sizeof(unsigned long long), h->stream));
-        HIPCHK(hipMemsetAsync(h->lstat.p, 0, h->lstat.n * sizeof(unsigned long long), h->stream));
-        HIPCHK(hipMemsetAsync(h->lprev.p, 0, h->lprev.n * sizeof(unsigned long long), h->stream));
+        {
+            static_assert(sizeof(CommitRec) % 4 == 0, "whole words");
+            const ClearList cl{{(unsigned*)h->tab.heavy.p, (unsigned*)h->rec.p, (unsigned*)h->cmax.p, (unsigned*)h->found.p,
+                                (unsigned*)h->lstat.p, (unsigned*)h->lprev.p},
+                               {h->tab.cap, sizeof(CommitRec) / 4, 2 * 2, h->found.n * 2, h->lstat.n * 2, h->lprev.n * 2}};
+            unsigned long long total = 0;
+            for (unsigned long long wds : cl.words) total += wds;
+            hipLaunchKernelGGL(k_clear_regions, dim3((unsigned)std::min<unsigned long long>((total + 255) / 256, 4096)), dim3(256), 0,
+                               h->stream, cl);
+        }
         if (c.m_rows > 0)
             hipLaunchKernelGGL(k_rebuild_scl, dim3((c.m_rows * h->d + 255) / 256), dim3(256), 0, h->stream, h->ctl.p, h->tab.view(),
                                c.m_rows, h->d, c.pow2, c.inv_k);
diff --git a/include/chronoclust_hip.h b/include/chronoclust_hip.h
--- a/include/chronoclust_hip.h
+++ b/include/chronoclust_hip.h
@@ -233,6 +233,7 @@
 } cc_relaxed_stats;
 int cc_get_relaxed_stats(cc_handle* h, cc_relaxed_stats* out);
 int cc_shard_rows(int32_t n, int32_t world, int32_t rank, int32_t unit, int32_t* lo, int32_t* hi);
+int32_t cc_list_order(const int32_t* kind, const int32_t* key, int32_t m, int32_t which_kind, int32_t* rows_out);
 int cc_set_shard_thresholds(cc_handle* h, int64_t min_row_dims, int32_t offline_min_rows);
 
 int cc_point_clusters(cc_handle* h, int32_t* out_idx);
```

Measured after the change: 79.27 million points/s (median of 6 runs). 1.7% higher.
